# iaomw/Tracer

Measured on AMD Instinct MI355X. Metric: Mrays/s at 1920x1080x64spp, higher is better.
Workload: dtype f32

## Files before the change

### include/tracer_test_hooks.h

```cpp
#ifndef TRACER_TEST_HOOKS_H
#define TRACER_TEST_HOOKS_H

#include "tracer_abi.h"

#ifdef __cplusplus
extern "C" {
#endif

trc_status trc_debug_profile(trc_ctx* ctx, uint64_t* out, uint32_t n_sites);
trc_status trc_sppm_hash_cells(trc_ctx* ctx, const float* cells , size_t n, float hash_scale, float* out );

trc_status trc_div_by_test(trc_ctx* ctx, const float* a, const float* b, size_t n, float* fast , float* plain );
trc_status trc_unary_test(trc_ctx* ctx, uint32_t op, uint32_t first_bits, uint64_t count, uint64_t* n_mismatch, uint32_t* first_mismatch);

trc_status trc_debug_denoise_state(trc_ctx* ctx, float* integrated, float* history, float* moments);

trc_status trc_texture_sample_test(trc_ctx* ctx, uint32_t index, const float* uv , size_t n, float* rgb );

trc_status trc_debug_env_tables(trc_ctx* ctx, float* weight, uint32_t* rows, uint32_t* marg, double* total, float* build_ms);
trc_status trc_env_light_test(trc_ctx* ctx, const uint32_t* draws , size_t n, float* dir_pdf ,
                              const float* dirs , size_t m, float* pdf );

trc_status trc_debug_mesh_light_tables(trc_ctx* ctx, uint32_t* alias , uint32_t* tri , float* pdfA ,
                                       double* total, uint32_t* n_lights);
trc_status trc_mesh_light_test(trc_ctx* ctx, const uint32_t* draws , const float* pos , size_t n, uint32_t* tri ,
                               float* out );

typedef struct trc_kernel_choice {
    uint32_t shape, variant, lds_resident, triangle_materials, strip, launches;
} trc_kernel_choice;
trc_status trc_debug_last_kernel(trc_ctx* ctx, trc_kernel_choice* out);

#ifdef __cplusplus
}
#endif
#endif
```

### tracer_amd/abi.py

```python
import ctypes as C

TRC_ABI_VERSION = 13
TRC_TILE = 16
TRC_MAX_BVH_DEPTH = 64
TREE_SAH, TREE_TRIANGLE_LEAVES = 1, 2
TRC_UNIQUE_ID_BYTES = 128
DT_U8, DT_U32, DT_F32 = 1, 3, 7
OP_SUM, OP_MAX, OP_MIN = 0, 2, 3

PRIM_SPHERE, PRIM_SQUARE, PRIM_CUBE, PRIM_TRIANGLE, PRIM_BVH, PRIM_UNKNOW = range(6)
(MAT_DIFFUSE, MAT_LAMBERT, MAT_ORENNAYAR, MAT_PLASTIC, MAT_METAL, MAT_GLASS,
 MAT_ISOTROPIC, MAT_DIELECTRIC, MAT_DEMOFOX, MAT_PBR, MAT_NIL) = range(11)
TEX_CONSTANT, TEX_CHECKER, TEX_NOISE, TEX_IMAGE = range(4)
INTEGRATOR_PATH, INTEGRATOR_MIS, INTEGRATOR_VOLUME = 0, 1, 2
MEDIUM_NIL, MEDIUM_HOMOGENEOUS, MEDIUM_GRIDDENSITY = 0, 1, 2
SCENE_CORNELL, SCENE_CORNELL_SPHERES, SCENE_CORNELL_MESH, SCENE_CORNELL_VOLUME = 0, 1, 2, 3
FLAG_COLLECT_STATS = 1
FLAG_FIXED_ORDER = 2
FLAG_SOBOL = 4
FLAG_SMALL_BLOCKS, FLAG_LARGE_BLOCKS = 8, 16
FLAG_ENV_LIGHT = 32
FLAG_MESH_LIGHTS = 64
TRACE_ANY_HIT, TRACE_PRODUCTION = 1, 2
SOBOL_DIMS, SOBOL_MATRIX_SIZE = 40, 52

SHARD_SEED_STRIDE = 0x9E3779B97F4A7C15


def shard_seed(seed, sample_group):
    return (int(seed) + int(sample_group) * SHARD_SEED_STRIDE) & 0xFFFFFFFFFFFFFFFF


OK = 0
ERR_INVALID_ARG, ERR_NO_DEVICE, ERR_HIP, ERR_NO_SCENE, ERR_NO_FRAME = -1, -2, -3, -4, -5
ERR_BVH_INVALID, ERR_UNSUPPORTED, ERR_RCCL, ERR_OOM = -6, -7, -8, -9


class float2(C.Structure):
    _fields_ = [("x", C.c_float), ("y", C.c_float)]


class float3(C.Structure):
    _fields_ = [("x", C.c_float), ("y", C.c_float), ("z", C.c_float), ("_pad", C.c_float)]


class float4(C.Structure):
    _fields_ = [("x", C.c_float), ("y", C.c_float), ("z", C.c_float), ("w", C.c_float)]


class float4x4(C.Structure):
    _fields_ = [("columns", float4 * 4)]


class AABB(C.Structure):
    _fields_ = [("mini", float3), ("maxi", float3)]


class BVH(C.Structure):
    _fields_ = [("parent", C.c_uint32), ("left", C.c_uint32), ("right", C.c_uint32), ("axis", C.c_uint32),
                ("pType", C.c_int32), ("pIndex", C.c_uint32), ("_pad", C.c_uint32 * 2), ("bBOX", AABB)]


class Sphere(C.Structure):
    _fields_ = [("radius", C.c_float), ("_pad0", C.c_uint32 * 3), ("center", float3),
                ("model_matrix", float4x4), ("normal_matrix", float4x4), ("inverse_matrix", float4x4),
                ("material", C.c_uint32), ("_pad1", C.c_uint32 * 3), ("boundingBOX", AABB)]


class Square(C.Structure):
    _fields_ = [("axis_i", C.c_uint8), ("axis_j", C.c_uint8), ("_pad0", C.c_uint8 * 6),
                ("range_i", float2), ("range_j", float2),
                ("axis_k", C.c_uint8), ("_pad1", C.c_uint8 * 3), ("value_k", C.c_float),
                ("model_matrix", float4x4), ("normal_matrix", float4x4), ("inverse_matrix", float4x4),
                ("material", C.c_uint32), ("_pad2", C.c_uint32 * 3), ("boundingBOX", AABB)]


class Cube(C.Structure):
    _fields_ = [("model_matrix", float4x4), ("normal_matrix", float4x4), ("inverse_matrix", float4x4),
                ("box", AABB), ("material", C.c_uint32), ("_pad", C.c_uint32 * 3)]


class TriangleVertex(C.Structure):
    _fields_ = [("v", C.c_float * 3), ("n", C.c_float * 3), ("uv", C.c_float * 2)]


class Pose(C.Structure):
    _fields_ = [("first", C.c_uint32), ("count", C.c_uint32), ("_pad", C.c_uint32 * 2),
                ("model_matrix", float4x4), ("normal_matrix", float4x4)]


class TextureInfo(C.Structure):
    _fields_ = [("type", C.c_int32), ("textureIndex", C.c_uint32), ("_pad", C.c_uint32 * 2), ("albedo", float3)]


class Image(C.Structure):
    _fields_ = [("width", C.c_uint32), ("height", C.c_uint32), ("rgb", C.POINTER(C.c_float))]


class Material(C.Structure):
    _fields_ = [("type", C.c_int32), ("medium", C.c_int32), ("specular", C.c_uint8), ("_pad0", C.c_uint8 * 3),
                ("eta", C.c_float), ("roughness", C.c_float), ("_pad1", C.c_uint32 * 3),
                ("textureInfo", TextureInfo)]


class Camera(C.Structure):
    _fields_ = [("lookFrom", float3), ("lookAt", float3), ("viewUp", float3),
                ("vfov", C.c_float), ("aspect", C.c_float), ("aperture", C.c_float), ("lenRadius", C.c_float),
                ("focus_dist", C.c_float), ("_pad", C.c_uint32 * 3),
                ("u", float3), ("v", float3), ("w", float3),
                ("vertical", float3), ("horizontal", float3), ("cornerLowLeft", float3)]


class PhotonRecord(C.Structure):
    _fields_ = [("flux", float3), ("normal", float3), ("position", float3), ("direction", float3),
                ("step", C.c_uint8), ("active", C.c_uint8), ("_pad", C.c_uint8 * 14)]


class CameraRecord(C.Structure):
    _fields_ = [("ratio", float3), ("position", float3), ("direction", float3),
                ("valid", C.c_uint8), ("_pad0", C.c_uint8 * 15), ("alternative", float3), ("flux", float3),
                ("radius", C.c_float), ("photonCount", C.c_uint32), ("_pad1", C.c_uint32 * 2)]


class Complex(C.Structure):
    _fields_ = [("tex_size", float2), ("view_size", float2), ("running_time", C.c_float),
                ("frame_count", C.c_uint32), ("_pad0", C.c_uint32 * 2), ("photonBox", AABB),
                ("photonBoxSize", float3), ("photonInitialRadius", C.c_float), ("photonHashScale", C.c_float),
                ("totalPhotonSum", C.c_float), ("framePhotonSum", C.c_uint32)]


PHOTON_HASHN = 512


class Scene(C.Structure):
    _fields_ = [("bvhList", C.POINTER(BVH)), ("n_bvh", C.c_uint32),
                ("sphereList", C.POINTER(Sphere)), ("n_sphere", C.c_uint32),
                ("squareList", C.POINTER(Square)), ("n_square", C.c_uint32),
                ("cubeList", C.POINTER(Cube)), ("n_cube", C.c_uint32),
                ("triList", C.POINTER(TriangleVertex)), ("n_vertex", C.c_uint32),
                ("idxList", C.POINTER(C.c_uint32)), ("n_index", C.c_uint32),
                ("materials", C.POINTER(Material)), ("n_material", C.c_uint32)]


class GridDensityInfo(C.Structure):
    _fields_ = [("sigma_a", C.c_float), ("sigma_s", C.c_float), ("sigma_t", C.c_float), ("g", C.c_float),
                ("invMaxDensity", C.c_float), ("nx", C.c_uint32), ("ny", C.c_uint32), ("nz", C.c_uint32)]


PBRT_MATTE, PBRT_PLASTIC, PBRT_METAL, PBRT_MIRROR, PBRT_GLASS, PBRT_OTHER = range(6)
PBRT_SHAPE_SPHERE, PBRT_SHAPE_TRIANGLEMESH, PBRT_SHAPE_DISK, PBRT_SHAPE_CYLINDER, PBRT_SHAPE_PLYMESH = 0, 3, 6, 7, 8
PBRT_SHAPE_CONE, PBRT_SHAPE_PARABOLOID, PBRT_SHAPE_HYPERBOLOID = 9, 10, 11
PBRT_TEX_NONE, PBRT_TEX_CHECKERBOARD, PBRT_TEX_OTHER = 0, 1, 2
PBRT_TRIANGLE_MATERIALS = 1


class PbrtInfo(C.Structure):
    _fields_ = [("camera_to_world", C.c_float * 16), ("fov", C.c_float), ("lensradius", C.c_float),
                ("focaldistance", C.c_float), ("perspective", C.c_uint32), ("xres", C.c_uint32), ("yres", C.c_uint32),
                ("n_shapes", C.c_uint32), ("n_unsupported_shapes", C.c_uint32), ("n_unsupported_materials", C.c_uint32),
                ("n_triangle_material_conflicts", C.c_uint32), ("mis_ready", C.c_uint32), ("n_unsupported_textures", C.c_uint32),
                ("n_instances", C.c_uint32)]


class PbrtShape(C.Structure):
    _fields_ = [("kind", C.c_int32), ("shape_to_world", C.c_float * 16), ("radius", C.c_float),
                ("n_vertices", C.c_uint32), ("n_indices", C.c_uint32), ("material", C.c_int32), ("color", C.c_float * 3),
                ("emitter", C.c_int32), ("L", C.c_float * 3), ("mapped_type", C.c_int32), ("mapped_index", C.c_uint32),
                ("mapped_material", C.c_uint32), ("zmin", C.c_float), ("zmax", C.c_float), ("innerradius", C.c_float),
                ("phimax", C.c_float), ("texture", C.c_int32), ("tex2", C.c_float * 3), ("p1", C.c_float * 3), ("p2", C.c_float * 3)]


class Params(C.Structure):
    _fields_ = [("spp", C.c_uint32), ("max_depth", C.c_uint32), ("integrator", C.c_uint32),
                ("frame0", C.c_uint32), ("tile_rank", C.c_uint32), ("tile_nranks", C.c_uint32),
                ("flags", C.c_uint32), ("view_height", C.c_uint32)]


class Ray(C.Structure):
    _fields_ = [("origin", C.c_float * 3), ("tmax", C.c_float), ("direction", C.c_float * 3), ("_pad", C.c_uint32)]


class Hit(C.Structure):
    _fields_ = [("hit", C.c_int32), ("pType", C.c_int32), ("pIndex", C.c_uint32), ("t", C.c_float),
                ("p", C.c_float * 3), ("gn", C.c_float * 3), ("sn", C.c_float * 3), ("uv", C.c_float * 2),
                ("material", C.c_uint32), ("PDF", C.c_float),
                ("n_descend", C.c_uint32), ("n_return", C.c_uint32), ("n_leaf", C.c_uint32)]


class GBufferTexel(C.Structure):
    _fields_ = [("depth", C.c_float), ("normal", C.c_float * 3), ("albedo", C.c_float * 3), ("id", C.c_uint32)]


class DenoiseParams(C.Structure):
    _fields_ = [("flags", C.c_uint32), ("iterations", C.c_uint32), ("alpha_color", C.c_float), ("alpha_moments", C.c_float),
                ("sigma_z", C.c_float), ("normal_exponent", C.c_uint32), ("sigma_l", C.c_float), ("min_history", C.c_uint32)]


GBUFFER_MISS = 0xFFFFFFFF
DENOISE_DEMODULATE = 1
DENOISE_ALBEDO_EPS = 0.001
DENOISE_MAX_ITERATIONS = 5


class KernelChoice(C.Structure):
    _fields_ = [("shape", C.c_uint32), ("variant", C.c_uint32), ("lds_resident", C.c_uint32), ("triangle_materials", C.c_uint32),
                ("strip", C.c_uint32), ("launches", C.c_uint32)]


KERNEL_SHAPES = ("one", "strip", "pwg", "dense")
KERNEL_VARIANTS = ("plain", "stats", "sobol", "tex", "env", "env_tex", "mesh", "mesh_tex")


class LaunchShape(C.Structure):
    _fields_ = [("entries", C.c_uint32), ("wave_slots", C.c_uint32), ("longest_entry_ms", C.c_double),
                ("sum_entries_ms", C.c_double), ("work_over_slots_ms", C.c_double), ("clock_mhz", C.c_double)]


class Stats(C.Structure):
    _fields_ = [("paths", C.c_uint64), ("rays", C.c_uint64), ("shaded", C.c_uint64),
                ("n_descend", C.c_uint64), ("n_return", C.c_uint64),
                ("n_leaf_sphere", C.c_uint64), ("n_leaf_square", C.c_uint64),
                ("n_leaf_cube", C.c_uint64), ("n_leaf_triangle", C.c_uint64),
                ("n_hit_triangle", C.c_uint64), ("n_hit_cube", C.c_uint64),
                ("launches", C.c_uint64), ("kernel_ms", C.c_double), ("schedule_ms", C.c_double)]

    def as_dict(self):
        return {n: getattr(self, n) for n, _ in self._fields_}


_EXPECTED_SIZES = {float2: 8, float3: 16, float4x4: 64, AABB: 32, BVH: 64, Sphere: 272, Square: 272, Cube: 240,
                   TriangleVertex: 32, Pose: 144, TextureInfo: 32, Material: 64, Camera: 176, Ray: 32, Params: 32, GBufferTexel: 32, DenoiseParams: 32,
                   PhotonRecord: 80, CameraRecord: 112, Complex: 96}
for _t, _n in _EXPECTED_SIZES.items():
    assert C.sizeof(_t) == _n, f"{_t.__name__}: ctypes size {C.sizeof(_t)} != ABI size {_n}"

DEVICE_SYMBOLS = [
    "trc_abi_version", "trc_build_flavor", "trc_has_test_hooks", "trc_status_string", "trc_last_error", "trc_create", "trc_destroy",
    "trc_upload_scene", "trc_upload_density", "trc_upload_scene_lbvh", "trc_upload_scene_sah", "trc_upload_scene_device", "trc_download_bvh", "trc_lbvh_info", "trc_set_camera", "trc_set_environment", "trc_set_environment_map", "trc_resize", "trc_seed",
    "trc_upload_rng", "trc_download_rng", "trc_upload_accum", "trc_download_accum", "trc_clear_accum", "trc_tonemap",
    "trc_render", "trc_synchronize", "trc_trace_rays", "trc_get_stats", "trc_reset_stats",
    "trc_sppm_init", "trc_sppm_frames", "trc_sppm_download",
    "trc_device_info", "trc_device_pci_bus_id", "trc_shard_seed", "trc_group_compose_samples", "trc_group_compose_samples_async", "trc_group_unique_id", "trc_group_init", "trc_group_reduce_accum", "trc_group_reduce_accum_async", "trc_group_allreduce_mean_accum", "trc_download_composed", "trc_group_finalize",
    "trc_group_set_collectives", "trc_debug_set", "trc_debug_block_costs", "trc_debug_launch_shape", "trc_debug_primary_replays",
    "trc_denoise_default_params", "trc_denoise", "trc_download_denoised", "trc_tonemap_denoised", "trc_download_gbuffer", "trc_denoise_reset",
    "trc_upload_textures", "trc_upload_triangle_materials", "trc_update_vertices", "trc_debug_refit_ms",
    "trc_pose_vertices", "trc_download_vertices", "trc_debug_pose_overflows",
]
HOOK_SYMBOLS = ["trc_debug_profile", "trc_sppm_hash_cells", "trc_div_by_test", "trc_unary_test", "trc_debug_denoise_state", "trc_texture_sample_test",
                "trc_debug_env_tables", "trc_env_light_test", "trc_debug_mesh_light_tables", "trc_mesh_light_test", "trc_debug_last_kernel"]
HOST_SYMBOLS = [
    "trc_host_build_node", "trc_host_build_tree", "trc_host_tree_depth", "trc_host_make_camera",
    "trc_host_prepare_camera", "trc_host_fill_rng", "trc_host_scene_create", "trc_host_scene_create_leaves", "trc_host_scene_destroy",
    "trc_host_scene_view", "trc_host_scene_load_pbrt", "trc_host_mesh_load_obj", "trc_host_mesh_load_pbrt", "trc_host_mesh_load_ply", "trc_host_load_hdr", "trc_host_mesh_make_ball", "trc_host_mesh_replicate", "trc_host_mesh_from_arrays",
    "trc_host_mesh_view", "trc_host_mesh_destroy", "trc_host_make_density_info", "trc_host_make_cloud",
    "trc_host_load_density_pbrt", "trc_host_free", "trc_host_write_png", "trc_host_sobol_matrices32",
    "trc_host_sobol_interval_tables", "trc_host_load_png", "trc_host_scene_load_pbrt_flags", "trc_host_scene_triangle_materials",
]
```

### tracer_amd/csrc/trc_ctx.hpp

```cpp
#pragma once

#include <hip/hip_runtime.h>

#include <initializer_list>
#include <string>
#include <utility>
#include <vector>

#include "tracer_abi.h"
#ifdef TRC_TEST_HOOKS
#include "tracer_test_hooks.h"
#endif
#include "dev_integrator.hpp"

using namespace trcdev;

extern __shared__ __attribute__((aligned(16))) uint32_t trc_smem[];

constexpr uint32_t kLaunchCodeShift = 25u;
constexpr uint32_t kLaunchIndexMask = (1u << kLaunchCodeShift) - 1u;
constexpr uint32_t kCostSlots = 84u;
constexpr uint32_t kPlanWords = 12u;

struct KScene {
    DScene sc;
    float root_box[6];
};

struct KRender {
    KScene ks;
    DCamera cam;
    float ambient[3];
    const float* env_rgb; uint32_t env_w, env_h;
    DFrame fr;
    uint32_t spp, max_depth, frame0;
    uint32_t view_height;
    const uint32_t* tiles;
    const float* density;
    trc_GridDensityInfo dinfo;
    const uint8_t* occupancy;
    unsigned long long* stats;
    uint32_t* stack_ovf;
    uint32_t* queue;
    uint32_t blk_shift;
    uint32_t n_tiles, strip;
    const uint32_t* order;
    const uint32_t* n_launch;
    uint32_t cost_div;
    uint32_t* block_cost;
    uint32_t cost_stride;
    const uint32_t* sobol32;
    const uint64_t* sobol_vdc;
    uint32_t sobol_m;
    const float* tex_texels;
    const uint4* tex_desc;
    uint32_t n_tex;
    uint32_t* memo;
    uint32_t replay;
    uint32_t replay_chain;
};

struct KRenderEnv {
    KRender kp;
    EnvLight el;
};

struct KRenderMesh {
    KRender kp;
    MeshLight ml;
};

struct KTrace {
    KScene ks;
    const trc_ray* rays;
    trc_hit* hits;
    uint32_t n;
};

__device__ __forceinline__ const uint32_t* stage_scene(const DScene& sc) {
    const uint4* src = reinterpret_cast<const uint4*>(sc.blob);
    uint4* dst = reinterpret_cast<uint4*>(trc_smem);
    const uint32_t n16 = sc.lds_dwords >> 2;
    for (uint32_t i = threadIdx.x; i < n16; i += kBlock) dst[i] = src[i];
    __syncthreads();
    return trc_smem;
}

__device__ __forceinline__ uint32_t* lane_stack(const DScene& sc) { return trc_smem + sc.lds_dwords + threadIdx.x; }
__device__ __forceinline__ uint32_t* lane_lvstack(const DScene& sc) { return trc_smem + sc.lds_dwords + sc.stack_lds * kBlock + threadIdx.x; }

__device__ __forceinline__ SceneRef make_scene_ref(const DScene& sc, const uint32_t* small_base) {
    SceneRef S;
    S.small_base = small_base;
    S.blob = sc.blob;
    S.off_nodes = sc.off_nodes; S.off_spheres = sc.off_spheres; S.off_squares = sc.off_squares;
    S.off_cubes = sc.off_cubes; S.off_materials = sc.off_materials;
    S.off_tripos = sc.off_tripos; S.off_triattr = sc.off_triattr;
    S.n_lds_nodes = sc.n_lds_nodes;
    S.stack_lds = sc.stack_lds;
    S.stack_cap = sc.stack_depth;
    S.ovf = nullptr;
    S.descend_min = sc.descend_min;
    return S;
}

constexpr uint32_t kStatRows = 1024;
constexpr uint32_t kStatRowStride = ((kStatCount + 3 * kProfCount + 15) / 16) * 16;
static_assert(kStatRowStride <= 64, "k_stats_sum sums a row with one 64-thread workgroup");
__device__ __forceinline__ unsigned long long* stat_row(unsigned long long* stats, uint32_t wave_index) {
    return stats + (size_t)(wave_index & (kStatRows - 1u)) * kStatRowStride;
}

__device__ __forceinline__ uint32_t wave_sum(uint32_t v) {
#pragma unroll
    for (int off = 32; off > 0; off >>= 1) v += __shfl_xor(v, off, 64);
    return v;
}


struct SppmState;
struct DenoiseState;

struct trc_ctx {
    int device = -1;
    hipStream_t stream = nullptr;
    hipEvent_t ev_start = nullptr, ev_stop = nullptr;
    std::string error;

    bool has_scene = false;
    KScene ks{};
    uint32_t* d_blob = nullptr;
    size_t blob_bytes = 0;
    bool lds_scene = false;
    bool lds_prefix_ok = false;
    uint32_t* d_stack_ovf = nullptr;
    size_t stack_ovf_bytes = 0;
    uint32_t* d_memo = nullptr;
    size_t memo_bytes = 0;
    uint32_t* d_queue = nullptr;
    trc_BVH* d_bvh_ref = nullptr;
    uint32_t n_bvh_ref = 0, lbvh_height = 0;
    float lbvh_build_ms = 0.0f;
    trc_TriangleVertex* d_verts = nullptr; uint32_t* d_idx = nullptr; uint32_t n_vertex = 0;
    uint32_t* d_refit_parent = nullptr;
    uint32_t* d_refit_refnode = nullptr;
    uint32_t* d_refit_arrive = nullptr;
    float* d_refit_root = nullptr;
    std::vector<uint32_t> refit_levels;
    float refit_ms = 0.0f;
    hipEvent_t refit_ev[3] = {nullptr, nullptr, nullptr};
    bool refit_pending = false;
    trc_TriangleVertex* d_rest = nullptr;
    trc_pose* d_pose_table = nullptr; size_t pose_table_bytes = 0;
    uint32_t pose_count_seen = 0;
    uint32_t pose_overflows = 0;
    bool refit_posed = false;
    float* d_density = nullptr;
    uint8_t* d_occupancy = nullptr;
    trc_GridDensityInfo dinfo{};

    bool has_camera = false;
    DCamera cam{};
    float ambient[3] = {0, 0, 0};
    float* d_envmap = nullptr; uint32_t env_w = 0, env_h = 0;
    uint32_t* d_sobol32 = nullptr; uint64_t* d_sobol_vdc = nullptr; uint32_t sobol_m = ~0u;
    float* d_tex_texels = nullptr; uint4* d_tex_desc = nullptr; uint32_t n_tex = 0; uint32_t scene_min_image = ~0u;
    bool tex_active() const { return scene_min_image < n_tex; }
    bool tri_materials = false;
    uint8_t* d_envl = nullptr; double envl_total = 0.0; float envl_build_ms = 0.0f;
    Light cost_light = Light::None;
    uint8_t* d_meshl = nullptr; bool mesh_built = false; uint32_t mesh_n_lights = 0; double mesh_total = 0.0;

    uint32_t width = 0, height = 0;
    uint32_t* d_rng = nullptr;
    float* d_accum = nullptr;

    uint32_t* d_tiles = nullptr;
    uint32_t* d_block_cost = nullptr;
    uint32_t* d_order_keys[2] = {nullptr, nullptr};
    uint32_t* d_order_vals[2] = {nullptr, nullptr};
    uint32_t* d_order_hist = nullptr;
    uint32_t* d_split = nullptr;
    uint32_t* d_whole = nullptr;
    uint32_t* d_cost_est = nullptr;
    uint32_t* d_qsplit = nullptr;
    uint32_t* d_qwhole = nullptr;
    uint32_t* d_swhole = nullptr;
    uint32_t* d_launch = nullptr;
    uint32_t* d_plan = nullptr;
    uint32_t* d_cost_scratch = nullptr;
    uint32_t* d_plan_gather = nullptr;
    uint32_t plan_streak = 0, plan_reused = 0, plan_n = 0, plan_wave_slots = 0, plan_grid_cap = 0; bool plan_split_mode = false;
    uint32_t launch_cap = 0;
    bool split_live = false;
    bool cost_quarters = false;
    bool cost_valid = false; uint32_t cost_strip = 1;
    uint32_t last_cost_div = 0, last_wave_slots = 0;
    struct LastKernel { uint32_t shape = 0, variant = 0, lds_resident = 0, tri_materials = 0, strip = 0, count = 0; } last_kernel;
    trc_params deferred{}; bool has_deferred = false; uint64_t deferred_calls = 0;
    int cost_head_age = 0;
    bool cost_fresh_next = false;
    uint32_t cost_integrator = 0xFFFFFFFFu;
    const uint32_t* d_stale_order = nullptr;
    const uint32_t* d_last_order = nullptr; uint32_t order_age = 0;
    int cu_count = 0;
    uint32_t n_tiles = 0, tiles_nranks = 0, tiles_rank = 0, tiles_view_height = 0, tiles_blk_shift = 3;

    unsigned long long* d_stats = nullptr;
    unsigned long long* d_stats_sum = nullptr;
    uint64_t launches = 0;
    double kernel_ms = 0.0;
    double schedule_ms = 0.0;
    std::vector<std::pair<hipEvent_t, hipEvent_t>> pending_sched;
    std::vector<std::pair<hipEvent_t, hipEvent_t>> pending;
    std::vector<hipEvent_t> event_pool;

    void* comm = nullptr;
    int nranks = 1, rank = 0;
    float* d_reduce_recv = nullptr;
    float* d_accum_alt = nullptr;
    float* d_composed = nullptr;
    hipStream_t comm_stream = nullptr;
    hipEvent_t ev_rendered = nullptr, ev_busy = nullptr, ev_busy_alt = nullptr;
    bool busy = false, busy_alt = false;
    float* d_shard_in = nullptr; float* d_shard_out = nullptr; size_t shard_px = 0; int shard_nranks = 0;
    float* d_shard_src = nullptr; hipEvent_t ev_snapshot_free = nullptr; bool snapshot_busy = false;

    SppmState* sppm = nullptr;
    DenoiseState* denoise = nullptr;

    trc_collectives coll{};
    bool coll_active = false;
    void* h_stage = nullptr;
    size_t h_stage_bytes = 0;
    uint32_t* h_readback = nullptr;
    char* h_xfer = nullptr;
    hipEvent_t ev_xfer[2] = {nullptr, nullptr};

    struct Knobs {
        int no_lds_fit = 0;
        int stack_lds_levels = 0;
        int strip_len = 0;
        int no_pwg = 0;
        int sppm_serial_camera = 0;
        int sppm_timing = 0;
        int force_blk_shift = 0;
        int no_split = 0;
        int no_cost_filter = 0;
        int no_cold_probe = 0;
        int probe_spp = 0;
        int no_plan_reuse = 0;
        int no_coalesce = 0;
        int no_dense = 0;
        int head_stages = 0;
        int descend_min = 0;
        int camera_policy = 0;
        int no_primary_replay = 0;
        int replay_min_lanes = 0;
        int replay_chain = 0;
        int mesh_light_pick = 1;
        int refit_single = 0;
        int strip_force = 0;
    } knobs;
    std::vector<const void*> lds_granted;

    bool grouped() const { return comm != nullptr || coll_active; }
};


inline trc_status trc_fail(trc_ctx* ctx, trc_status s, const std::string& msg) {
    if (ctx) ctx->error = msg;
    return s;
}
#define HIP_TRY(ctx, expr)                                                                 \
    do {                                                                                   \
        hipError_t e_ = (expr);                                                            \
        if (e_ != hipSuccess)                                                              \
            return trc_fail(ctx, e_ == hipErrorOutOfMemory ? TRC_ERR_OOM : TRC_ERR_HIP,     \
                            std::string(#expr) + ": " + hipGetErrorString(e_));            \
    } while (0)

#define TRC_TRY(expr)                                                                      \
    do {                                                                                   \
        const trc_status s_ = (expr);                                                      \
        if (s_ != TRC_OK) return s_;                                                       \
    } while (0)

struct DevBuf {
    void* p = nullptr;
    DevBuf() = default;
    DevBuf(DevBuf&& o) noexcept : p(o.release()) {}
    DevBuf(const DevBuf&) = delete;
    DevBuf& operator=(const DevBuf&) = delete;
    ~DevBuf() { (void)hipFree(p); }
    trc_status alloc(trc_ctx* ctx, size_t bytes, const char* what) {
        if (hipMalloc(&p, bytes) == hipSuccess) return TRC_OK;
        p = nullptr;
        (void)hipGetLastError();
        return trc_fail(ctx, TRC_ERR_OOM, std::string("hipMalloc ") + what);
    }
    template <class T> T* as() const { return static_cast<T*>(p); }
    void* release() { void* q = p; p = nullptr; return q; }
};

struct DevBufs {
    std::vector<DevBuf> bufs;
    template <class T> trc_status alloc(trc_ctx* ctx, T** out, size_t count, const char* what) {
        bufs.emplace_back();
        TRC_TRY(bufs.back().alloc(ctx, (count ? count : 1) * sizeof(T), what));
        *out = bufs.back().as<T>();
        return TRC_OK;
    }
};

template <class T>
inline trc_status trc_grow_buffer(trc_ctx* ctx, T*& buf, size_t& have, size_t need, const char* msg) {
    if (need <= have) return TRC_OK;
    HIP_TRY(ctx, hipStreamSynchronize(ctx->stream));
    (void)hipFree(buf); buf = nullptr;
    have = 0;
    if (hipMalloc((void**)&buf, need) != hipSuccess) return trc_fail(ctx, TRC_ERR_OOM, msg);
    have = need;
    return TRC_OK;
}

struct IdBlob { char internal[TRC_UNIQUE_ID_BYTES]; };
struct Rccl {
    void* handle = nullptr;
    bool ready = false;
    int (*GetUniqueId)(void*) = nullptr;
    int (*CommInitRank)(void**, int, IdBlob, int) = nullptr;
    int (*Reduce)(const void*, void*, size_t, int, int, int, void*, hipStream_t) = nullptr;
    int (*AllReduce)(const void*, void*, size_t, int, int, void*, hipStream_t) = nullptr;
    int (*AllGather)(const void*, void*, size_t, int, void*, hipStream_t) = nullptr;
    int (*Send)(const void*, size_t, int, int, void*, hipStream_t) = nullptr;
    int (*Recv)(void*, size_t, int, int, void*, hipStream_t) = nullptr;
    int (*GroupStart)() = nullptr;
    int (*GroupEnd)() = nullptr;
    int (*CommDestroy)(void*) = nullptr;
    const char* (*GetErrorString)(int) = nullptr;
};
extern Rccl g_rccl;
bool trc_load_rccl(std::string& err);
constexpr int kNcclUint8 = 1, kNcclUint32 = 3, kNcclFloat = 7, kNcclSum = 0, kNcclMax = 2, kNcclMin = 3;

trc_status trc_coll_reduce(trc_ctx* ctx, void* buf, size_t count, int dtype, int op, int root, hipStream_t st, const char* what);
trc_status trc_coll_allreduce(trc_ctx* ctx, void* buf, size_t count, int dtype, int op, hipStream_t st, const char* what);
trc_status trc_coll_allgather(trc_ctx* ctx, void* buf, size_t bytes_per_rank, hipStream_t st, const char* what);

constexpr size_t kXferChunk = 4u << 20;
trc_status trc_copy_to_host(trc_ctx* ctx, void* host, const void* dev, size_t bytes, hipStream_t st);
trc_status trc_copy_to_device(trc_ctx* ctx, void* dev, const void* host, size_t bytes, hipStream_t st);
struct trc_read_item { void* host; const void* dev; size_t bytes; };
trc_status trc_read_to_host(trc_ctx* ctx, hipStream_t st, const char* what, std::initializer_list<trc_read_item> items);

trc_status trc_ensure_tiles(trc_ctx* ctx, uint32_t nranks, uint32_t rank, uint32_t view_height = 0, uint32_t blk_shift = 3);
size_t trc_dyn_lds_bytes(const trc_ctx* ctx, bool stats);
void trc_sort_pairs24(hipStream_t st, uint32_t* keys[2], uint32_t* vals[2], uint32_t* hist, uint32_t* digit_base, uint32_t n, int* result);
uint32_t trc_sort_hist_words(uint32_t n);
trc_status trc_tonemap_plane(trc_ctx* ctx, const float* plane, uint8_t* rgba8, float* exposure_out);
trc_status trc_flush(trc_ctx* ctx);
hipEvent_t trc_get_event(trc_ctx* ctx);
struct TimedSection {
    trc_ctx* ctx; hipStream_t st; hipEvent_t e0, e1;
    TimedSection(trc_ctx* c, hipStream_t s) : ctx(c), st(s), e0(trc_get_event(c)), e1(trc_get_event(c)) { if (e0 && e1) (void)hipEventRecord(e0, st); }
    ~TimedSection() { if (e0) ctx->event_pool.push_back(e0); if (e1) ctx->event_pool.push_back(e1); }
    void stop() { if (e0 && e1) (void)hipEventRecord(e1, st); }
    float ms() const { float v = 0.0f; return e0 && e1 && hipEventElapsedTime(&v, e0, e1) == hipSuccess ? v : 0.0f; }
};
void trc_sppm_release(trc_ctx* ctx);
void trc_denoise_release(trc_ctx* ctx);
inline uint32_t trc_scene_min_image(const trc_scene* s) {
    uint32_t m = ~0u;
    for (uint32_t i = 0; i < s->n_material; ++i)
        if (s->materials[i].textureInfo.type == TRC_TEX_IMAGE && s->materials[i].textureInfo.textureIndex < m) m = s->materials[i].textureInfo.textureIndex;
    return m;
}
void trc_denoise_invalidate(trc_ctx* ctx);
trc_status trc_env_light_build(trc_ctx* ctx);
void trc_env_light_free(trc_ctx* ctx);
EnvLight trc_env_light_view(const trc_ctx* ctx);
trc_status trc_mesh_light_build(trc_ctx* ctx);
void trc_mesh_light_free(trc_ctx* ctx);
MeshLight trc_mesh_light_view(const trc_ctx* ctx);
constexpr size_t kReadbackBytes = 1024;
inline trc_status trc_readback_alloc(trc_ctx* ctx) {
    if (!ctx->h_readback) HIP_TRY(ctx, hipHostMalloc((void**)&ctx->h_readback, kReadbackBytes, hipHostMallocDefault));
    return TRC_OK;
}
trc_status trc_refit_settle_pending(trc_ctx* ctx);
inline trc_status trc_refit_settle(trc_ctx* ctx) { return ctx->refit_pending ? trc_refit_settle_pending(ctx) : TRC_OK; }
void trc_refit_free(trc_ctx* ctx);
void trc_sppm_order_after_camera(trc_ctx* ctx);

inline void trc_forget_costs(trc_ctx* ctx) { ctx->cost_valid = false; ctx->d_last_order = nullptr; ctx->d_stale_order = nullptr; }
inline void trc_picture_changed(trc_ctx* ctx) { trc_denoise_invalidate(ctx); }
enum SceneChange { kSceneReplaced, kSceneMaterials, kSceneVerticesMoved };
void trc_scene_changed(trc_ctx* ctx, SceneChange kind);
void trc_release_scene(trc_ctx* ctx);
void trc_adopt_scene(trc_ctx* ctx, KScene ks, const trc_scene* s);
void trc_release_frame(trc_ctx* ctx);
void trc_release_tiles(trc_ctx* ctx);
void trc_collect_finished_events(trc_ctx* ctx);
trc_status trc_read_stats_sum(trc_ctx* ctx, unsigned long long* h, size_t count);
```

### tracer_amd/csrc/trc_hooks.hip

```cpp
#include <hip/hip_runtime.h>

#include <string>

#include "trc_ctx.hpp"

extern "C" int trc_has_test_hooks(void) {
#ifdef TRC_TEST_HOOKS
    return 1;
#else
    return 0;
#endif
}

#ifdef TRC_TEST_HOOKS
__global__ void __launch_bounds__(256) k_div_by_test(const float* a, const float* b, uint32_t n, float* fast, float* plain) {
    const uint32_t i = blockIdx.x * 256u + threadIdx.x;
    if (i >= n) return;
    const float av = a[i], bv = b[i];
    const GuardedDivBy d = guarded_div_by(bv);
    const F3 q = guarded_div(f3(av, -av, av * 0.75f), d);
    fast[3 * i] = q.x; fast[3 * i + 1] = q.y; fast[3 * i + 2] = q.z;
    plain[3 * i] = av / bv; plain[3 * i + 1] = -av / bv; plain[3 * i + 2] = (av * 0.75f) / bv;
}

__global__ void __launch_bounds__(256) k_unary_test(uint32_t op, uint32_t first, uint64_t count, unsigned long long* out) {
    unsigned long long bad = 0, first_bad = ~0ull;
    for (uint64_t i = (uint64_t)blockIdx.x * 256u + threadIdx.x; i < count; i += (uint64_t)gridDim.x * 256u) {
        const uint32_t bits = first + (uint32_t)i;
        const float x = __uint_as_float(bits);
        float a, b;
        if (op == 0u) { a = rcp_cr(x); b = 1.0f / x; }
        else if (op == 1u) { a = sqrt_cr(x); b = sqrtf(x); }
#if TRC_WAVE_GUARDS
        else if (op == 3u) { a = div_const(x, div_by_pi()); b = x / kPi; }
        else if (op == 4u) { a = div_const(x, div_by_sqr001()); b = x / (0.01f * 0.01f); }
        else if (op == 5u) { a = div_const(x, div_by_sqr002()); b = x / (0.02f * 0.02f); }
        else if (op == 6u) { a = div_const(x, div_by_sqr01()); b = x / (0.1f * 0.1f); }
#endif
        else { a = rsqrt_cr(x); b = 1.0f / sqrtf(x); }
        const bool same = __float_as_uint(a) == __float_as_uint(b) || (a != a && b != b);
        if (!same) { bad++; first_bad = min(first_bad, (unsigned long long)bits); }
    }
    if (bad) { atomicAdd(&out[0], bad); atomicMin(&out[1], first_bad); }
}

extern "C" {
trc_status trc_debug_profile(trc_ctx* ctx, uint64_t* out, uint32_t n_sites) {
    TRC_TRY(trc_flush(ctx));
    if (!ctx || !out) return TRC_ERR_INVALID_ARG;
    HIP_TRY(ctx, hipSetDevice(ctx->device));
    unsigned long long h[kStatCount + 3 * kProfCount];
    TRC_TRY(trc_read_stats_sum(ctx, h, kStatCount + 3 * kProfCount));
    for (uint32_t i = 0; i < n_sites && i < (uint32_t)kProfCount; ++i)
        for (int k = 0; k < 3; ++k) out[3 * i + k] = h[kStatCount + 3 * i + k];
    return TRC_OK;
}

__global__ void __launch_bounds__(256) k_texture_sample_test(const float* texels, const uint4* desc, uint32_t n_tex, uint32_t index,
                                                             const float* uv, uint32_t n, float* rgb) {
    const uint32_t i = blockIdx.x * 256u + threadIdx.x;
    if (i >= n) return;
    TexTable tt; tt.texels = texels; tt.desc = desc; tt.n = n_tex;
    F2 p; p.x = uv[2 * i]; p.y = uv[2 * i + 1];
    const F3 c = image_sample(tt, index, p);
    rgb[3 * i] = c.x; rgb[3 * i + 1] = c.y; rgb[3 * i + 2] = c.z;
}
trc_status trc_texture_sample_test(trc_ctx* ctx, uint32_t index, const float* uv, size_t n, float* rgb) {
    TRC_TRY(trc_flush(ctx));
    if (!ctx || (n && (!uv || !rgb))) return TRC_ERR_INVALID_ARG;
    if (index >= ctx->n_tex) return trc_fail(ctx, TRC_ERR_INVALID_ARG, "trc_texture_sample_test: no such image");
    if (n == 0) return TRC_OK;
    if (n > 0x7FFFFFFFu / 3u) return trc_fail(ctx, TRC_ERR_INVALID_ARG, "trc_texture_sample_test: too many pairs in one call");
    HIP_TRY(ctx, hipSetDevice(ctx->device));
    DevBuf d;
    TRC_TRY(d.alloc(ctx, n * 5 * sizeof(float), "texture sample test"));
    float *d_uv = d.as<float>(), *d_rgb = d_uv + 2 * n;
    TRC_TRY(trc_copy_to_device(ctx, d_uv, uv, n * 8, ctx->stream));
    hipLaunchKernelGGL(k_texture_sample_test, dim3((unsigned)((n + 255) / 256)), dim3(256), 0, ctx->stream,
                       ctx->d_tex_texels, ctx->d_tex_desc, ctx->n_tex, index, d_uv, (uint32_t)n, d_rgb);
    const hipError_t e = hipGetLastError();
    if (e != hipSuccess) return trc_fail(ctx, TRC_ERR_HIP, std::string("trc_texture_sample_test: ") + hipGetErrorString(e));
    return trc_copy_to_host(ctx, rgb, d_rgb, n * 12, ctx->stream);
}

trc_status trc_debug_last_kernel(trc_ctx* ctx, trc_kernel_choice* out) {
    TRC_TRY(trc_flush(ctx));
    if (!ctx || !out) return TRC_ERR_INVALID_ARG;
    const trc_ctx::LastKernel& k = ctx->last_kernel;
    out->shape = k.shape; out->variant = k.variant; out->lds_resident = k.lds_resident; out->triangle_materials = k.tri_materials;
    out->strip = k.strip; out->launches = k.count;
    return TRC_OK;
}

trc_status trc_div_by_test(trc_ctx* ctx, const float* a, const float* b, size_t n, float* fast, float* plain) {
    if (!ctx || (n && (!a || !b || !fast || !plain))) return TRC_ERR_INVALID_ARG;
    if (n == 0) return TRC_OK;
    if (n > 0x7FFFFFFFu / 3u) return trc_fail(ctx, TRC_ERR_INVALID_ARG, "trc_div_by_test: too many pairs in one call");
    HIP_TRY(ctx, hipSetDevice(ctx->device));
    DevBuf d;
    TRC_TRY(d.alloc(ctx, n * 8 * sizeof(float), "div_by test"));
    float *d_a = d.as<float>(), *d_b = d_a + n, *d_fast = d_a + 2 * n, *d_plain = d_a + 5 * n;
    TRC_TRY(trc_copy_to_device(ctx, d_a, a, n * 4, ctx->stream));
    TRC_TRY(trc_copy_to_device(ctx, d_b, b, n * 4, ctx->stream));
    hipLaunchKernelGGL(k_div_by_test, dim3((unsigned)((n + 255) / 256)), dim3(256), 0, ctx->stream, d_a, d_b, (uint32_t)n, d_fast, d_plain);
    const hipError_t e = hipGetLastError();
    if (e != hipSuccess) return trc_fail(ctx, TRC_ERR_HIP, std::string("trc_div_by_test: ") + hipGetErrorString(e));
    TRC_TRY(trc_copy_to_host(ctx, fast, d_fast, n * 12, ctx->stream));
    return trc_copy_to_host(ctx, plain, d_plain, n * 12, ctx->stream);
}

trc_status trc_unary_test(trc_ctx* ctx, uint32_t op, uint32_t first_bits, uint64_t count, uint64_t* n_mismatch, uint32_t* first_mismatch) {
    if (!ctx || !n_mismatch || op > 6u || count > (1ull << 32)) return TRC_ERR_INVALID_ARG;
    HIP_TRY(ctx, hipSetDevice(ctx->device));
    DevBuf buf;
    TRC_TRY(buf.alloc(ctx, 16, "unary test"));
    unsigned long long* const d = buf.as<unsigned long long>();
    unsigned long long h[2] = {0ull, ~0ull};
    TRC_TRY(trc_copy_to_device(ctx, d, h, 16, ctx->stream));
    if (count) hipLaunchKernelGGL(k_unary_test, dim3(ctx->cu_count * 16), dim3(256), 0, ctx->stream, op, first_bits, count, d);
    TRC_TRY(trc_read_to_host(ctx, ctx->stream, "trc_unary_test", {{h, d, 16}}));
    *n_mismatch = h[0];
    if (first_mismatch) *first_mismatch = (uint32_t)h[1];
    return TRC_OK;
}

}
#endif
```

### tracer_amd/csrc/trc_render_config.hpp

```cpp
#pragma once

#include "trc_ctx.hpp"

#ifndef TRC_MIS_HYBRID
#define TRC_MIS_HYBRID 1
#endif
#ifndef TRC_VOLUME_HYBRID
#define TRC_VOLUME_HYBRID 0
#endif
constexpr bool hybrid_stack(int integrator) {
    return integrator == TRC_INTEGRATOR_PATH || (integrator == TRC_INTEGRATOR_MIS ? TRC_MIS_HYBRID != 0 : TRC_VOLUME_HYBRID != 0);
}
#ifndef TRC_DEFER_LDS
#define TRC_DEFER_LDS 0
#endif
#ifndef TRC_DEFER_GLOBAL
#define TRC_DEFER_GLOBAL 1
#endif

#ifndef TRC_PATH_WAVES
#define TRC_PATH_WAVES 5
#endif
#ifndef TRC_PATH_WAVES_DENSE
#define TRC_PATH_WAVES_DENSE 6
#endif
#ifndef TRC_DENSE_MIN_BLOCKS_PER_SLOT
#define TRC_DENSE_MIN_BLOCKS_PER_SLOT 4
#endif
#ifndef TRC_PATH_WAVES_GLOBAL
#define TRC_PATH_WAVES_GLOBAL 7
#endif
#ifndef TRC_MIS_WAVES
#define TRC_MIS_WAVES 8
#endif
#ifndef TRC_MIS_WAVES_LDS
#define TRC_MIS_WAVES_LDS 8
#endif
#ifndef TRC_VOLUME_WAVES
#define TRC_VOLUME_WAVES 4
#endif
#ifndef TRC_PWG_WAVES_PATH
#define TRC_PWG_WAVES_PATH 4
#endif
#ifndef TRC_PWG_PER_CU_PATH
#define TRC_PWG_PER_CU_PATH 7
#endif
#ifndef TRC_PWG_WAVES_MIS
#define TRC_PWG_WAVES_MIS 16
#endif
#ifndef TRC_PWG_PER_CU_MIS
#define TRC_PWG_PER_CU_MIS 2
#endif
#ifndef TRC_PWG_WAVES_VOLUME
#define TRC_PWG_WAVES_VOLUME 16
#endif
#ifndef TRC_PWG_PER_CU_VOLUME
#define TRC_PWG_PER_CU_VOLUME 1
#endif
#ifndef TRC_STRIP_PATH_WAVES
#define TRC_STRIP_PATH_WAVES 4
#endif
constexpr int pwg_waves(int integrator) { return integrator == TRC_INTEGRATOR_PATH ? TRC_PWG_WAVES_PATH : (integrator == TRC_INTEGRATOR_MIS ? TRC_PWG_WAVES_MIS : TRC_PWG_WAVES_VOLUME); }
enum : uint32_t { kParkCachedX = 0, kParkCachedY, kParkCachedZ, kParkU, kParkV, kParkSample, kParkRays, kParkShaded, kParkPx, kParkPy };
#ifndef TRC_PARK_PATH
#define TRC_PARK_PATH 8
#endif
#ifndef TRC_PARK_MIS
#define TRC_PARK_MIS 0
#endif
#ifndef TRC_PARK_VOLUME
#define TRC_PARK_VOLUME 10
#endif
#ifndef TRC_PARK_DENSE
#define TRC_PARK_DENSE 0
#endif
constexpr uint32_t pwg_park_rows(int integrator) { return integrator == TRC_INTEGRATOR_PATH ? TRC_PARK_PATH : (integrator == TRC_INTEGRATOR_MIS ? TRC_PARK_MIS : TRC_PARK_VOLUME); }
static_assert((TRC_PARK_PATH == 0 || TRC_PARK_PATH == 8 || TRC_PARK_PATH == 10) && (TRC_PARK_MIS == 0 || TRC_PARK_MIS == 8 || TRC_PARK_MIS == 10) &&
              (TRC_PARK_VOLUME == 0 || TRC_PARK_VOLUME == 8 || TRC_PARK_VOLUME == 10) && (TRC_PARK_DENSE == 0 || TRC_PARK_DENSE == 8 || TRC_PARK_DENSE == 10), "park rows: 0, 8 or 10");
enum : uint32_t { kMemoPx = 0, kMemoPy, kMemoPz, kMemoNx, kMemoNy, kMemoNz, kMemoTag, kMemoMat, kMemoU, kMemoV };
constexpr uint32_t kMemoNone = 0xFFFFFFFFu;
constexpr uint32_t kMemoSameSide = 0x80000000u;
#ifndef TRC_REPLAY_DENSE
#define TRC_REPLAY_DENSE 8
#endif
#ifndef TRC_REPLAY_DENSE_GLOBAL
#define TRC_REPLAY_DENSE_GLOBAL 0
#endif
#ifndef TRC_REPLAY_PWG_PATH
#define TRC_REPLAY_PWG_PATH 10
#endif
#ifndef TRC_REPLAY_MIN_LANES
#define TRC_REPLAY_MIN_LANES 1
#endif
#ifndef TRC_REPLAY_CHAIN
#define TRC_REPLAY_CHAIN 1
#endif
static_assert((TRC_REPLAY_DENSE == 0 || TRC_REPLAY_DENSE == 8 || TRC_REPLAY_DENSE == 10) && (TRC_REPLAY_PWG_PATH == 0 || TRC_REPLAY_PWG_PATH == 10), "memo rows: 0, 8 or 10 (10 wherever image textures may be live)");
constexpr uint32_t dense_lds_rows() { return (uint32_t)TRC_PARK_DENSE + (TRC_REPLAY_DENSE_GLOBAL ? 0u : (uint32_t)TRC_REPLAY_DENSE); }
constexpr uint32_t pwg_memo_rows(int integrator) { return integrator == TRC_INTEGRATOR_PATH ? (uint32_t)TRC_REPLAY_PWG_PATH : 0u; }
#ifndef TRC_PWG_STACK_LDS_PATH
#define TRC_PWG_STACK_LDS_PATH (TRC_PARK_PATH == 10 ? 10 : (TRC_PARK_PATH == 8 ? 12 : 16))
#endif
#ifndef TRC_PWG_STACK_LDS_MIS
#define TRC_PWG_STACK_LDS_MIS 8
#endif
#ifndef TRC_PWG_STACK_LDS_VOLUME
#define TRC_PWG_STACK_LDS_VOLUME 16
#endif
constexpr uint32_t pwg_stack_lds_levels(int integrator) { return integrator == TRC_INTEGRATOR_MIS ? TRC_PWG_STACK_LDS_MIS : (integrator == TRC_INTEGRATOR_PATH ? TRC_PWG_STACK_LDS_PATH : TRC_PWG_STACK_LDS_VOLUME); }
constexpr int pwg_per_cu(int integrator) { return integrator == TRC_INTEGRATOR_PATH ? TRC_PWG_PER_CU_PATH : (integrator == TRC_INTEGRATOR_MIS ? TRC_PWG_PER_CU_MIS : TRC_PWG_PER_CU_VOLUME); }

constexpr int render_waves(bool lds, bool stats, int integrator) {
    return stats ? 1 : integrator == TRC_INTEGRATOR_VOLUME ? TRC_VOLUME_WAVES
                     : integrator == TRC_INTEGRATOR_MIS ? (lds ? TRC_MIS_WAVES_LDS : TRC_MIS_WAVES) : (lds ? TRC_PATH_WAVES : TRC_PATH_WAVES_GLOBAL);
}
constexpr int strip_waves(int integrator) { return integrator == TRC_INTEGRATOR_VOLUME ? 3 : (integrator == TRC_INTEGRATOR_PATH ? TRC_STRIP_PATH_WAVES : 4); }
constexpr int pwg_simd_waves(int integrator) { return pwg_waves(integrator) * pwg_per_cu(integrator) / 4; }

enum RenderArgs { kArgsPlain, kArgsEnv, kArgsMesh };
struct RenderKernel {
    const void* fn;
    int waves;
    RenderArgs args;
};
inline RenderKernel render_kernel(void (*fn)(KRender), int waves) { return {reinterpret_cast<const void*>(fn), waves, kArgsPlain}; }
inline RenderKernel render_kernel(void (*fn)(KRenderEnv), int waves) { return {reinterpret_cast<const void*>(fn), waves, kArgsEnv}; }
inline RenderKernel render_kernel(void (*fn)(KRenderMesh), int waves) { return {reinterpret_cast<const void*>(fn), waves, kArgsMesh}; }
enum RenderVariant { kVariantPlain, kVariantStats, kVariantSobol, kVariantTex, kVariantEnv, kVariantEnvTex, kVariantMesh, kVariantMeshTex, kVariants };
struct RenderKernels {
    RenderKernel one[kVariants];
    RenderKernel strip[kVariants];
    RenderKernel pwg[kVariants];
};
extern const RenderKernels render_lds_path, render_lds_mis, render_lds_volume, render_mem_path, render_mem_mis, render_mem_volume;
extern const RenderKernel render_dense;
namespace trimat {
extern const RenderKernels render_lds_path, render_lds_mis, render_lds_volume, render_mem_path, render_mem_mis, render_mem_volume;
extern const RenderKernel render_dense;
}
```

### tracer_amd/csrc/trc_render_kernels.hpp

```cpp
#pragma once

#include <hip/hip_runtime.h>

#include "trc_render_config.hpp"

#if TRC_TRIANGLE_MATERIALS
#define TRC_RENDER_NS_BEGIN namespace trimat {
#define TRC_RENDER_NS_END }
#else
#define TRC_RENDER_NS_BEGIN
#define TRC_RENDER_NS_END
#endif
TRC_RENDER_NS_BEGIN

template <bool TEX, class CX>
__device__ __forceinline__ void set_ctx_tex(CX& cx, const KRender& kp) {
    if constexpr (TEX) { cx.tex.texels = kp.tex_texels; cx.tex.desc = kp.tex_desc; cx.tex.n = kp.n_tex; }
}
template <Light LIGHT, class CX>
__device__ __forceinline__ void set_ctx_light(CX& cx, const LightTables<LIGHT>* tables) {
    if constexpr (LIGHT != Light::None) cx.light = *tables;
}
template <bool SOBOL, bool TEX, Light LIGHT>
__device__ __forceinline__ void fill_path_ctx(PathCtxOf<TEX, LIGHT>& cx, const KRender& kp, const DScene& sc, const uint32_t* small_base,
                                              uint32_t* stack, uint32_t* lvstack, const LightTables<LIGHT>* tables) {
    cx.S = make_scene_ref(sc, small_base);
    cx.root_min = f3(kp.ks.root_box[0], kp.ks.root_box[1], kp.ks.root_box[2]);
    cx.root_max = f3(kp.ks.root_box[3], kp.ks.root_box[4], kp.ks.root_box[5]);
    cx.sh.mats = small_base + sc.off_materials;
    set_ctx_tex<TEX>(cx, kp);
    set_ctx_light<LIGHT>(cx, tables);
    cx.ambient = f3(kp.ambient[0], kp.ambient[1], kp.ambient[2]);
    cx.env.rgb = kp.env_rgb; cx.env.w = kp.env_w; cx.env.h = kp.env_h;
    cx.stack = stack;
    cx.lvstack = lvstack;
    cx.max_depth = kp.max_depth;
    cx.density = kp.density;
    cx.dinfo = kp.dinfo;
    cx.occupancy = kp.occupancy;
    if (SOBOL) {
        cx.sobol32 = kp.sobol32; cx.sobol_vdc = kp.sobol_vdc;
        cx.sobol_m = kp.sobol_m; cx.sobol_res = 1u << kp.sobol_m;
    }
}
template <bool LDS, bool STATS, int INTEGRATOR, bool SOBOL, bool HYB, int PARK = 0, bool TEX = false, Light LIGHT = Light::None, int MEMO = 0, class COUNT = uint32_t>
__device__ __forceinline__ void render_block(const KRender& kp, const DScene& sc, const uint32_t* small_base, uint32_t* stack, uint32_t* lvstack,
                                             uint32_t* ovf, uint32_t* park, const uint32_t slot, const uint32_t lane,
                                             COUNT& n_rays, COUNT& n_shaded, uint32_t& n_paths, TravCounters& cnt,
                                             const LightTables<LIGHT>* tables = nullptr, uint32_t* memo = nullptr) {
    static_assert(MEMO == 0 || (INTEGRATOR == TRC_INTEGRATOR_PATH && !STATS && !SOBOL && LIGHT == Light::None), "primary replay: tracePath production kernels");
    static_assert(MEMO == 0 || MEMO == 10 || !TEX, "an image texture reads rec.uv: 10 memo rows");
    uint32_t replays = 0;
    const uint64_t t_start = clock64();
    const uint32_t entry = kp.order ? kp.order[slot] : slot;
    const uint32_t index = entry & kLaunchIndexMask, code = entry >> kLaunchCodeShift;
    if (index >= kp.n_tiles) return;
    const uint32_t tile = kp.tiles[index];
    const uint32_t part = code >= 21u ? (code - 21u) >> 2 : (code >= 5u ? code - 5u : 0u);
    const uint32_t quarter = code >= 5u ? part >> 2 : (code ? code - 1u : 0u);
    const uint32_t bs = code >= 21u ? 0u : (code >= 5u ? 1u : (code ? 2u : kp.blk_shift));
    const uint32_t pixel = code >= 21u ? (code - 21u) & 3u : 0u;
    const uint32_t qx = code ? ((quarter & 1u) << 2) + (code >= 5u ? (part & 1u) << 1 : 0u) + (pixel & 1u) : 0u;
    const uint32_t qy = code ? ((quarter >> 1) << 2) + (code >= 5u ? ((part >> 1) & 1u) << 1 : 0u) + (pixel >> 1) : 0u;
    const uint32_t px = ((tile & 0xFFFFu) << kp.blk_shift) + qx + (lane & ((1u << bs) - 1u));
    const uint32_t py = ((tile >> 16) << kp.blk_shift) + qy + (lane >> bs);
    const uint32_t W = kp.fr.width, H = kp.fr.height;
    const bool active = lane < (1u << (2u * bs)) && px < W && py < H;
    const uint32_t canon = index * kp.cost_stride + (code ? code - 1u : 0u);

    if (active) {
        PathCtxOf<TEX, LIGHT> cx;
        fill_path_ctx<SOBOL, TEX, LIGHT>(cx, kp, sc, small_base, stack, lvstack, tables);
        cx.S.ovf = ovf;
        if (SOBOL) { cx.sobol_xy[0] = px; cx.sobol_xy[1] = py % kp.view_height; }

        F3 cached_r = f3(0);
        float u_r = 0, v_r = 0;
        uint32_t s_r = 0;
        size_t pix_r = 0;
        auto row_f = [&](uint32_t r) { return __uint_as_float(park[r * kBlock]); };
        auto put_f = [&](uint32_t r, float x) { park[r * kBlock] = __float_as_uint(x); };
        auto get_cached = [&]() { if constexpr (PARK) return f3(row_f(kParkCachedX), row_f(kParkCachedY), row_f(kParkCachedZ)); else return cached_r; };
        auto set_cached = [&](F3 c) { if constexpr (PARK) { put_f(kParkCachedX, c.x); put_f(kParkCachedY, c.y); put_f(kParkCachedZ, c.z); } else cached_r = c; };
        auto get_sample = [&]() { if constexpr (PARK) return park[kParkSample * kBlock]; else return s_r; };
        auto set_sample = [&](uint32_t s) { if constexpr (PARK) park[kParkSample * kBlock] = s; else s_r = s; };
        uint4 texel;
        {
            const size_t pix = (size_t)py * W + px;
            texel = reinterpret_cast<const uint4*>(kp.fr.rng)[pix];
            const float4 acc = reinterpret_cast<const float4*>(kp.fr.accum)[pix];
            const float u = (float)px / (float)W;
            const float v = (float)(py % kp.view_height) / (float)kp.view_height;
            set_cached(f3(acc.x, acc.y, acc.z));
            set_sample(0u);
            if constexpr (PARK) { put_f(kParkU, u); put_f(kParkV, v); }
            if constexpr (PARK >= 10) { park[kParkPx * kBlock] = px; park[kParkPy * kBlock] = py; }
            else { u_r = u; v_r = v; pix_r = pix; }
        }

        PathState ps;
        Pcg rng;
        uint64_t state_after_cast = 0;
        const bool replay_on = MEMO != 0 && kp.replay != 0u;
        bool first = replay_on, have = false, terminal = false;
        auto memo_f = [&](uint32_t r) { return __uint_as_float(memo[r * kBlock]); };
        auto at_eye = [&](const F3& o) {
            return __float_as_uint(o.x) == __float_as_uint(kp.cam.lookFrom[0]) && __float_as_uint(o.y) == __float_as_uint(kp.cam.lookFrom[1]) &&
                   __float_as_uint(o.z) == __float_as_uint(kp.cam.lookFrom[2]);
        };
        auto begin_sample = [&](uint32_t s) {
            const float u = PARK ? row_f(kParkU) : u_r, v = PARK ? row_f(kParkV) : v_r;
            path_begin(ps, cast_ray(kp.cam, u, v, rng), kp.max_depth);
            if constexpr (MEMO != 0) {
                if (replay_on && s != 0u) {
                    const uint32_t mat = memo[kMemoMat * kBlock];
                    if (mat != kMemoNone) {
                        if (at_eye(ps.ray.o)) {
                            const uint32_t tag = memo[kMemoTag * kBlock];
                            if (tag == kTagNone) terminal = true;
                            else {
                                ps.rec.p = f3(memo_f(kMemoPx), memo_f(kMemoPy), memo_f(kMemoPz));
                                ps.rec.gn = f3(memo_f(kMemoNx), memo_f(kMemoNy), memo_f(kMemoNz));
                                ps.rec.sn = (mat & kMemoSameSide) ? ps.rec.gn : -ps.rec.gn;
                                ps.rec.material = mat & ~kMemoSameSide;
                                ps.rec.tag = tag;
                                if constexpr (MEMO >= 10) { ps.rec.uv.x = memo_f(kMemoU); ps.rec.uv.y = memo_f(kMemoV); }
                                have = true;
                            }
                            bump(n_rays);
                        } else {
                            memo[kMemoMat * kBlock] = kMemoNone; memo[kMemoTag * kBlock] = s - 1u;
                        }
                    }
                }
            }
            if (SOBOL) {
                state_after_cast = rng.state;
                ps.sobol_index = sobol_interval_to_index(cx, (uint64_t)(kp.frame0 + s));
                ps.sobol_dim = 0;
            }
        };
        bool alive = kp.spp > 0;
        if (alive) {
            rng.state = ((uint64_t)texel.z << 32) | texel.w;
            rng.inc = ((uint64_t)texel.x << 32) | texel.y;
            begin_sample(0u);
        }
        auto finish_sample = [&](F3 color) {
            ProfScope<STATS> scope(cnt, kProfFinish);
            for (;;) {
                const bool bad = is_inf(color.x) || is_nan(color.x) || is_inf(color.y) || is_nan(color.y) ||
                                 is_inf(color.z) || is_nan(color.z);
                if (bad) color = f3(0);
                uint32_t s = get_sample();
                const uint32_t frame = kp.frame0 + s;
                set_cached(div_shared(get_cached() * (float)frame + color, (float)(frame + 1)));
                if (SOBOL) rng.state = state_after_cast;
                if constexpr (!PARK) {
                    texel.y = (uint32_t)rng.state; texel.x = (uint32_t)(rng.state >> 32);
                    texel.w = (uint32_t)rng.inc;   texel.z = (uint32_t)(rng.inc >> 32);
                    n_paths++;
                }
                ++s;
                set_sample(s);
                if (s == kp.spp) {
                    alive = false;
                } else {
                    if constexpr (PARK) { const uint64_t t = rng.state; rng.state = rng.inc; rng.inc = t; }
                    else {
                        rng.state = ((uint64_t)texel.z << 32) | texel.w;
                        rng.inc = ((uint64_t)texel.x << 32) | texel.y;
                    }
                    begin_sample(s);
                }
                if constexpr (MEMO != 0) {
                    if (terminal) { terminal = false; color = f3(memo_f(kMemoPx), memo_f(kMemoPy), memo_f(kMemoPz)); continue; }
                }
                break;
            }
        };
        auto memo_store = [&](bool hitted) {
            uint32_t mat = kMemoNone, tag = 0u;
            bool ends = false;
            if (at_eye(ps.ray.o)) {
                ends = !hitted || mat_type(cx.sh, ps.rec.material) == kMatDiffuse;
                if (ends) { mat = 0u; tag = kTagNone; }
                else {
                    const bool uv_read = MEMO < 10 && (ps.rec.tag >> kTagIndexBits) >= 2u && mat_tex(cx.sh, ps.rec.material) == kTexChecker;
                    if (!uv_read && ps.rec.material < kMemoSameSide - 1u) {
                        const bool same = __float_as_uint(ps.rec.sn.x) == __float_as_uint(ps.rec.gn.x);
                        mat = ps.rec.material | (same ? kMemoSameSide : 0u); tag = ps.rec.tag;
                        memo[kMemoPx * kBlock] = __float_as_uint(ps.rec.p.x); memo[kMemoPy * kBlock] = __float_as_uint(ps.rec.p.y);
                        memo[kMemoPz * kBlock] = __float_as_uint(ps.rec.p.z);
                        memo[kMemoNx * kBlock] = __float_as_uint(ps.rec.gn.x); memo[kMemoNy * kBlock] = __float_as_uint(ps.rec.gn.y);
                        memo[kMemoNz * kBlock] = __float_as_uint(ps.rec.gn.z);
                        if constexpr (MEMO >= 10) { memo[kMemoU * kBlock] = __float_as_uint(ps.rec.uv.x); memo[kMemoV * kBlock] = __float_as_uint(ps.rec.uv.y); }
                    }
                }
            }
            memo[kMemoMat * kBlock] = mat; memo[kMemoTag * kBlock] = tag;
            return ends;
        };
        uint32_t drained = 0;
        while (alive) {
            ProfScope<STATS> loop_scope(cnt, kProfLoop);
            constexpr bool kVolume = INTEGRATOR == TRC_INTEGRATOR_VOLUME;
            constexpr int kDefer = STATS ? 0 : (LDS ? TRC_DEFER_LDS : TRC_DEFER_GLOBAL);
            bool hitted = true;
            bool drain = false, ends = false;
            if constexpr (MEMO != 0) {
                drain = (uint32_t)__popcll(__ballot(have)) >= kp.replay && drained < kp.replay_chain && replay_on;
                drained = drain ? drained + 1u : 0u;
            }
            if (!drain && !have && !(kVolume && TRC_TRACK_SLICE > 0 && ps.tracking)) {
                bump(n_rays);
                hitted = scene_hit<LDS, STATS, false, false, kVolume, HYB, kDefer>(cx.S, cx.root_min, cx.root_max, ps.ray, ps.rec, FLT_MAX,
                                                                                  cx.stack, cx.lvstack, cnt);
                if constexpr (MEMO != 0) {
                    if (first) { ends = memo_store(hitted); first = false; }
                }
            }
            if (!drain || have) {
                have = false;
                F3 color;
                const bool finished = (INTEGRATOR == TRC_INTEGRATOR_PATH)
                                          ? path_step<STATS, SOBOL, TEX>(cx, ps, hitted, rng, cnt, n_shaded, color)
                                          : mis_step<LDS, STATS, kVolume, SOBOL, HYB, TEX, LIGHT>(cx, ps, hitted, rng, cnt, n_rays, n_shaded, color);
                if constexpr (MEMO != 0) {
                    if (ends) { memo[kMemoPx * kBlock] = __float_as_uint(color.x); memo[kMemoPy * kBlock] = __float_as_uint(color.y); memo[kMemoPz * kBlock] = __float_as_uint(color.z); }
                }
                if (finished) finish_sample(color);
            }
        }
        if constexpr (MEMO != 0) {
            if (replay_on) replays = memo[kMemoMat * kBlock] != kMemoNone ? kp.spp - 1u : memo[kMemoTag * kBlock];
        }
        if constexpr (PARK) {
            n_paths += kp.spp;
            texel.y = (uint32_t)rng.state; texel.x = (uint32_t)(rng.state >> 32);
            texel.w = (uint32_t)rng.inc;   texel.z = (uint32_t)(rng.inc >> 32);
        }
        const F3 cached = get_cached();
        size_t pix = pix_r;
        if constexpr (PARK >= 10) pix = (size_t)park[kParkPy * kBlock] * W + park[kParkPx * kBlock];
        else if constexpr (PARK != 0) {
            const uint32_t entry2 = kp.order ? *reinterpret_cast<const volatile uint32_t*>(kp.order + slot) : slot;
            const uint32_t code2 = entry2 >> kLaunchCodeShift;
            const uint32_t tile2 = *reinterpret_cast<const volatile uint32_t*>(kp.tiles + (entry2 & kLaunchIndexMask));
            const uint32_t part2 = code2 >= 21u ? (code2 - 21u) >> 2 : (code2 >= 5u ? code2 - 5u : 0u);
            const uint32_t quarter2 = code2 >= 5u ? part2 >> 2 : (code2 ? code2 - 1u : 0u);
            const uint32_t bs2 = code2 >= 21u ? 0u : (code2 >= 5u ? 1u : (code2 ? 2u : kp.blk_shift));
            const uint32_t pixel2 = code2 >= 21u ? (code2 - 21u) & 3u : 0u;
            const uint32_t qx2 = code2 ? ((quarter2 & 1u) << 2) + (code2 >= 5u ? (part2 & 1u) << 1 : 0u) + (pixel2 & 1u) : 0u;
            const uint32_t qy2 = code2 ? ((quarter2 >> 1) << 2) + (code2 >= 5u ? ((part2 >> 1) & 1u) << 1 : 0u) + (pixel2 >> 1) : 0u;
            pix = (size_t)(((tile2 >> 16) << kp.blk_shift) + qy2 + (lane >> bs2)) * W + ((tile2 & 0xFFFFu) << kp.blk_shift) + qx2 + (lane & ((1u << bs2) - 1u));
        }
        float4 out; out.x = cached.x; out.y = cached.y; out.z = cached.z; out.w = 1.0f;
        reinterpret_cast<float4*>(kp.fr.accum)[pix] = out;
        reinterpret_cast<uint4*>(kp.fr.rng)[pix] = texel;
    }

    if (lane == 0) kp.block_cost[canon] = (uint32_t)min((unsigned long long)(clock64() - t_start) / kp.cost_div, 0xFFFFFFull);
    if constexpr (MEMO != 0) {
        const uint32_t r_replays = wave_sum(replays);
        if (lane == 0 && r_replays) atomicAdd(&stat_row(kp.stats, slot)[kStatReplays], (unsigned long long)r_replays);
    }
}

template <bool LDS, bool STATS, int INTEGRATOR, bool SOBOL, int PARK = 0, bool TEX = false, Light LIGHT = Light::None, int MEMO = 0, bool MEMO_GLOBAL = false>
__device__ __forceinline__ void render_workgroup(const KRender& kp, const LightTables<LIGHT>* tables = nullptr) {
    if (kp.n_launch && blockIdx.x >= *kp.n_launch) return;
    const DScene& sc = kp.ks.sc;
    const uint32_t* small_base = stage_scene(sc);
    uint32_t* stack = lane_stack(sc);
    uint32_t* lvstack = lane_lvstack(sc);

    const uint32_t lane = threadIdx.x;
    uint32_t n_rays = 0, n_shaded = 0, n_paths = 0;
    TravCounters cnt;
    counters_zero(cnt);
    constexpr bool kHybridStack = !LDS && !STATS && hybrid_stack(INTEGRATOR);
    uint32_t* ovf = kHybridStack ? kp.stack_ovf + (size_t)blockIdx.x * sc.stack_ovf_rows * kBlock + lane : nullptr;
    uint32_t* memo = nullptr;
    if constexpr (MEMO != 0 && MEMO_GLOBAL) memo = kp.memo + (size_t)blockIdx.x * MEMO * kBlock + lane;
    else if constexpr (MEMO != 0) memo = stack + (sc.stack_lds + PARK) * kBlock;
    if constexpr (PARK != 0) {
        uint32_t* park = stack + sc.stack_lds * kBlock;
        park[kParkRays * kBlock] = 0u; park[kParkShaded * kBlock] = 0u;
        LdsCount c_rays{park + kParkRays * kBlock}, c_shaded{park + kParkShaded * kBlock};
        render_block<LDS, STATS, INTEGRATOR, SOBOL, kHybridStack, PARK, TEX, LIGHT, MEMO>(kp, sc, small_base, stack, lvstack, ovf, park, blockIdx.x, lane, c_rays, c_shaded, n_paths, cnt, tables, memo);
        n_rays = park[kParkRays * kBlock]; n_shaded = park[kParkShaded * kBlock];
    } else
    render_block<LDS, STATS, INTEGRATOR, SOBOL, kHybridStack, 0, TEX, LIGHT, MEMO>(kp, sc, small_base, stack, lvstack, ovf, nullptr, blockIdx.x, lane, n_rays, n_shaded, n_paths, cnt, tables, memo);

    uint32_t r_paths = wave_sum(n_paths), r_rays = wave_sum(n_rays), r_shaded = wave_sum(n_shaded);
    unsigned long long* const stats = stat_row(kp.stats, blockIdx.x);
    if (lane == 0) {
        atomicAdd(&stats[kStatPaths], (unsigned long long)r_paths);
        atomicAdd(&stats[kStatRays], (unsigned long long)r_rays);
        atomicAdd(&stats[kStatShaded], (unsigned long long)r_shaded);
    }
    if (STATS) {
        uint32_t v[8] = {cnt.n_descend, cnt.n_return, cnt.leaf[0], cnt.leaf[1], cnt.leaf[2], cnt.leaf[3],
                         cnt.hit_triangle, cnt.hit_cube};
        const int slot[8] = {kStatDescend, kStatReturn, kStatLeafSphere, kStatLeafSquare, kStatLeafCube,
                             kStatLeafTriangle, kStatHitTriangle, kStatHitCube};
#pragma unroll
        for (int i = 0; i < 8; ++i) {
            uint32_t r = wave_sum(v[i]);
            if (lane == 0) atomicAdd(&stats[slot[i]], (unsigned long long)r);
        }
        for (int i = 0; i < kProfCount; ++i) {
            uint32_t rl = wave_sum(cnt.prof_lane[i]), rw = wave_sum(cnt.prof_wave[i]);
            unsigned long long rc = cnt.prof_cycles[i];
#pragma unroll
            for (int off = 32; off > 0; off >>= 1) rc += __shfl_xor(rc, off);
            if (lane == 0) {
                atomicAdd(&stats[kStatCount + 3 * i], (unsigned long long)rl);
                atomicAdd(&stats[kStatCount + 3 * i + 1], (unsigned long long)rw);
                atomicAdd(&stats[kStatCount + 3 * i + 2], rc);
            }
        }
    }
}
template <bool LDS, bool STATS, int INTEGRATOR, bool SOBOL>
__global__ void __launch_bounds__(kBlock, render_waves(LDS, STATS, INTEGRATOR)) k_render(const KRender kp) { render_workgroup<LDS, STATS, INTEGRATOR, SOBOL>(kp); }
template <bool LDS, int INTEGRATOR>
__global__ void __launch_bounds__(kBlock, render_waves(LDS, false, INTEGRATOR)) k_render_tex(const KRender kp) { render_workgroup<LDS, false, INTEGRATOR, false, 0, true>(kp); }
template <bool LDS, int INTEGRATOR, bool TEX>
__global__ void __launch_bounds__(kBlock, render_waves(LDS, false, INTEGRATOR)) k_render_env(const KRenderEnv kpe) {
    render_workgroup<LDS, false, INTEGRATOR, false, 0, TEX, Light::Env>(kpe.kp, &kpe.el);
}
template <bool LDS, int INTEGRATOR, bool TEX>
__global__ void __launch_bounds__(kBlock, render_waves(LDS, false, INTEGRATOR)) k_render_mesh(const KRenderMesh kpm) {
    render_workgroup<LDS, false, INTEGRATOR, false, 0, TEX, Light::Mesh>(kpm.kp, &kpm.ml);
}

template <int INTEGRATOR, bool SOBOL>
__global__ void __launch_bounds__(64 * pwg_waves(INTEGRATOR), pwg_simd_waves(INTEGRATOR)) k_render_pwg(const KRender kp) {
    constexpr bool TEX = false;
    constexpr Light LIGHT = Light::None;
    const void* const tables = nullptr;
#include "trc_render_pwg_body.inc"
}
template <int INTEGRATOR>
__global__ void __launch_bounds__(64 * pwg_waves(INTEGRATOR), pwg_simd_waves(INTEGRATOR)) k_render_pwg_tex(const KRender kp) {
    constexpr bool SOBOL = false, TEX = true;
    constexpr Light LIGHT = Light::None;
    const void* const tables = nullptr;
#include "trc_render_pwg_body.inc"
}
template <int INTEGRATOR, bool TEX>
__global__ void __launch_bounds__(64 * pwg_waves(INTEGRATOR), pwg_simd_waves(INTEGRATOR)) k_render_pwg_env(const KRenderEnv kpe) {
    constexpr bool SOBOL = false;
    constexpr Light LIGHT = Light::Env;
    const KRender& kp = kpe.kp;
    const EnvLight* const tables = &kpe.el;
#include "trc_render_pwg_body.inc"
}

template <int INTEGRATOR, bool TEX>
__global__ void __launch_bounds__(64 * pwg_waves(INTEGRATOR), pwg_simd_waves(INTEGRATOR)) k_render_pwg_mesh(const KRenderMesh kpm) {
    constexpr bool SOBOL = false;
    constexpr Light LIGHT = Light::Mesh;
    const KRender& kp = kpm.kp;
    const MeshLight* const tables = &kpm.ml;
#include "trc_render_pwg_body.inc"
}

template <bool LDS, int INTEGRATOR, bool SOBOL>
__global__ void __launch_bounds__(kBlock, strip_waves(INTEGRATOR)) k_render_strip(const KRender kp) {
    constexpr bool TEX = false;
    constexpr Light LIGHT = Light::None;
    const void* const tables = nullptr;
#include "trc_render_strip_body.inc"
}
template <bool LDS, int INTEGRATOR>
__global__ void __launch_bounds__(kBlock, strip_waves(INTEGRATOR)) k_render_strip_tex(const KRender kp) {
    constexpr bool SOBOL = false, TEX = true;
    constexpr Light LIGHT = Light::None;
    const void* const tables = nullptr;
#include "trc_render_strip_body.inc"
}
template <bool LDS, int INTEGRATOR, bool TEX>
__global__ void __launch_bounds__(kBlock, strip_waves(INTEGRATOR)) k_render_strip_env(const KRenderEnv kpe) {
    constexpr bool SOBOL = false;
    constexpr Light LIGHT = Light::Env;
    const KRender& kp = kpe.kp;
    const EnvLight* const tables = &kpe.el;
#include "trc_render_strip_body.inc"
}

template <bool LDS, int INTEGRATOR, bool TEX>
__global__ void __launch_bounds__(kBlock, strip_waves(INTEGRATOR)) k_render_strip_mesh(const KRenderMesh kpm) {
    constexpr bool SOBOL = false;
    constexpr Light LIGHT = Light::Mesh;
    const KRender& kp = kpm.kp;
    const MeshLight* const tables = &kpm.ml;
#include "trc_render_strip_body.inc"
}

template <bool LDS, int INTEGRATOR>
inline RenderKernels render_kernels() {
    constexpr bool kSobol = INTEGRATOR != TRC_INTEGRATOR_VOLUME;
    RenderKernels t{};
    t.one[kVariantPlain] = render_kernel(&k_render<LDS, false, INTEGRATOR, false>, render_waves(LDS, false, INTEGRATOR));
    t.one[kVariantStats] = render_kernel(&k_render<LDS, true, INTEGRATOR, false>, render_waves(LDS, true, INTEGRATOR));
    t.one[kVariantTex] = render_kernel(&k_render_tex<LDS, INTEGRATOR>, render_waves(LDS, false, INTEGRATOR));
    t.strip[kVariantPlain] = render_kernel(&k_render_strip<LDS, INTEGRATOR, false>, strip_waves(INTEGRATOR));
    t.strip[kVariantTex] = render_kernel(&k_render_strip_tex<LDS, INTEGRATOR>, strip_waves(INTEGRATOR));
    if constexpr (kSobol) {
        t.one[kVariantSobol] = render_kernel(&k_render<LDS, false, INTEGRATOR, true>, render_waves(LDS, false, INTEGRATOR));
        t.strip[kVariantSobol] = render_kernel(&k_render_strip<LDS, INTEGRATOR, true>, strip_waves(INTEGRATOR));
    }
    if constexpr (!LDS) {
        t.pwg[kVariantPlain] = render_kernel(&k_render_pwg<INTEGRATOR, false>, pwg_simd_waves(INTEGRATOR));
        t.pwg[kVariantTex] = render_kernel(&k_render_pwg_tex<INTEGRATOR>, pwg_simd_waves(INTEGRATOR));
        if constexpr (kSobol) t.pwg[kVariantSobol] = render_kernel(&k_render_pwg<INTEGRATOR, true>, pwg_simd_waves(INTEGRATOR));
    }
    if constexpr (INTEGRATOR == TRC_INTEGRATOR_MIS) {
        t.one[kVariantEnv] = render_kernel(&k_render_env<LDS, INTEGRATOR, false>, render_waves(LDS, false, INTEGRATOR));
        t.one[kVariantEnvTex] = render_kernel(&k_render_env<LDS, INTEGRATOR, true>, render_waves(LDS, false, INTEGRATOR));
        t.strip[kVariantEnv] = render_kernel(&k_render_strip_env<LDS, INTEGRATOR, false>, strip_waves(INTEGRATOR));
        t.strip[kVariantEnvTex] = render_kernel(&k_render_strip_env<LDS, INTEGRATOR, true>, strip_waves(INTEGRATOR));
        if constexpr (!LDS) {
            t.pwg[kVariantEnv] = render_kernel(&k_render_pwg_env<INTEGRATOR, false>, pwg_simd_waves(INTEGRATOR));
            t.pwg[kVariantEnvTex] = render_kernel(&k_render_pwg_env<INTEGRATOR, true>, pwg_simd_waves(INTEGRATOR));
        }
        t.one[kVariantMesh] = render_kernel(&k_render_mesh<LDS, INTEGRATOR, false>, render_waves(LDS, false, INTEGRATOR));
        t.one[kVariantMeshTex] = render_kernel(&k_render_mesh<LDS, INTEGRATOR, true>, render_waves(LDS, false, INTEGRATOR));
        t.strip[kVariantMesh] = render_kernel(&k_render_strip_mesh<LDS, INTEGRATOR, false>, strip_waves(INTEGRATOR));
        t.strip[kVariantMeshTex] = render_kernel(&k_render_strip_mesh<LDS, INTEGRATOR, true>, strip_waves(INTEGRATOR));
        if constexpr (!LDS) {
            t.pwg[kVariantMesh] = render_kernel(&k_render_pwg_mesh<INTEGRATOR, false>, pwg_simd_waves(INTEGRATOR));
            t.pwg[kVariantMeshTex] = render_kernel(&k_render_pwg_mesh<INTEGRATOR, true>, pwg_simd_waves(INTEGRATOR));
        }
    }
    return t;
}
TRC_RENDER_NS_END
```

### tracer_amd/csrc/trc_render_pass.hip

```cpp
#include <hip/hip_runtime.h>

#include <algorithm>
#include <cstring>
#include <string>
#include <vector>

#include "trc_launch.hpp"

static size_t dyn_lds_bytes(const DScene& sc, bool stats) {
    size_t dwords = sc.lds_dwords + (size_t)sc.stack_lds * kBlock * (stats ? 2u : 1u);
    return dwords * 4;
}
size_t trc_dyn_lds_bytes(const trc_ctx* ctx, bool stats) { return dyn_lds_bytes(ctx->ks.sc, stats); }

constexpr uint32_t kStackLdsLevels = 16;
static void set_hybrid_stack(DScene& sc, uint32_t levels) {
    sc.stack_lds = std::min(sc.stack_depth, std::max(1u, levels));
    sc.stack_ovf_rows = sc.stack_depth - sc.stack_lds;
}
static void plan_launch_lds(const trc_ctx* ctx, DScene& sc, uint32_t waves_per_simd, bool hybrid) {
    const uint32_t levels = ctx->knobs.stack_lds_levels > 0 ? (uint32_t)ctx->knobs.stack_lds_levels : kStackLdsLevels;
    if (hybrid) set_hybrid_stack(sc, ctx->knobs.no_lds_fit ? std::max(levels, sc.stack_depth) : levels);
    if (ctx->knobs.no_lds_fit) return;
    if (!ctx->lds_prefix_ok) return;
    const uint32_t per_wg = ((160u * 1024u / 4u) / (4u * waves_per_simd)) & ~127u;
    const uint32_t stack = sc.stack_lds * kBlock;
    uint32_t room = std::max(per_wg > stack ? per_wg - stack : 0u, sc.off_nodes + kNodeDwords);
    room = std::min(room, kLdsSceneBytes / 4);
    sc.n_lds_nodes = std::min(sc.n_nodes, (room - sc.off_nodes) / kNodeDwords);
    sc.lds_dwords = sc.off_nodes + sc.n_lds_nodes * kNodeDwords;
}

static bool plan_pwg_lds(const trc_ctx* ctx, DScene& sc, uint32_t waves, uint32_t per_cu, bool hybrid, uint32_t default_levels, uint32_t park_rows) {
    uint32_t levels = ctx->knobs.stack_lds_levels > 0 ? (uint32_t)ctx->knobs.stack_lds_levels : default_levels;
    const uint32_t per_wg = ((160u * 1024u / 4u) / per_cu) & ~127u;
    for (;; --levels) {
        DScene t = sc;
        if (hybrid) set_hybrid_stack(t, levels);
        const uint32_t stacks = waves * (t.stack_lds + park_rows) * kBlock;
        if (per_wg >= stacks + t.off_nodes + kNodeDwords) {
            t.n_lds_nodes = std::min(t.n_nodes, (per_wg - stacks - t.off_nodes) / kNodeDwords);
            t.lds_dwords = t.off_nodes + t.n_lds_nodes * kNodeDwords;
            sc = t;
            return true;
        }
        if (!hybrid || levels <= 6u || ctx->knobs.stack_lds_levels > 0) return false;
    }
}

namespace {

trc_status ensure_sobol_tables(trc_ctx* ctx, uint32_t m) {
    if (!ctx->d_sobol_vdc) {
        std::vector<uint32_t> m32(TRC_SOBOL_DIMS * TRC_SOBOL_MATRIX_SIZE);
        trc_sobol_matrices32(m32.data());
        if (!ctx->d_sobol32) HIP_TRY(ctx, hipMalloc((void**)&ctx->d_sobol32, m32.size() * sizeof(uint32_t)));
        TRC_TRY(trc_copy_to_device(ctx, ctx->d_sobol32, m32.data(), m32.size() * sizeof(uint32_t), ctx->stream));
        HIP_TRY(ctx, hipMalloc((void**)&ctx->d_sobol_vdc, 2 * TRC_SOBOL_MATRIX_SIZE * sizeof(uint64_t)));
        ctx->sobol_m = ~0u;
    }
    if (ctx->sobol_m != m) {
        uint64_t tb[2 * TRC_SOBOL_MATRIX_SIZE] = {};
        if (m != 0 && trc_sobol_interval_tables(m, tb, tb + TRC_SOBOL_MATRIX_SIZE) != 0)
            return trc_fail(ctx, TRC_ERR_UNSUPPORTED, "Sobol interval tables");
        HIP_TRY(ctx, hipStreamSynchronize(ctx->stream));
        TRC_TRY(trc_copy_to_device(ctx, ctx->d_sobol_vdc, tb, sizeof(tb), ctx->stream));
        ctx->sobol_m = m;
    }
    return TRC_OK;
}

const RenderKernels& render_family(bool lds_scene, uint32_t integrator, bool tri_materials) {
    static const RenderKernels* const lds[3] = {&render_lds_path, &render_lds_mis, &render_lds_volume};
    static const RenderKernels* const mem[3] = {&render_mem_path, &render_mem_mis, &render_mem_volume};
    static const RenderKernels* const lds_tm[3] = {&trimat::render_lds_path, &trimat::render_lds_mis, &trimat::render_lds_volume};
    static const RenderKernels* const mem_tm[3] = {&trimat::render_mem_path, &trimat::render_mem_mis, &trimat::render_mem_volume};
    return *(tri_materials ? (lds_scene ? lds_tm : mem_tm) : (lds_scene ? lds : mem))[integrator];
}

hipError_t launch_render(trc_ctx* ctx, const RenderLaunch& r) {
    const void* const fn = r.kern.fn;
    if (r.lds > 64 * 1024 && std::find(ctx->lds_granted.begin(), ctx->lds_granted.end(), fn) == ctx->lds_granted.end()) {
        const hipError_t e = hipFuncSetAttribute(fn, hipFuncAttributeMaxDynamicSharedMemorySize, (int)(160 * 1024));
        if (e != hipSuccess) return e;
        ctx->lds_granted.push_back(fn);
    }
    KRenderEnv kpe;
    KRenderMesh kpm;
    void* params = const_cast<KRender*>(&r.kp);
    if (r.kern.args == kArgsEnv) { kpe.kp = r.kp; kpe.el = r.el; params = &kpe; }
    if (r.kern.args == kArgsMesh) { kpm.kp = r.kp; kpm.ml = r.ml; params = &kpm; }
    void* args[] = {params};
    const hipError_t e = hipLaunchKernel(fn, dim3(r.grid), dim3(r.block), args, r.lds, ctx->stream);
    const hipError_t last = hipGetLastError();
    return e != hipSuccess ? e : last;
}

}

static trc_status render_pass(trc_ctx* ctx, const trc_params* p, bool inner);

constexpr uint32_t kColdHeadSpp = 8;
static trc_status render_check(trc_ctx* ctx, const trc_params* p, uint32_t* sobol_m = nullptr) {
    if (!ctx || !p) return TRC_ERR_INVALID_ARG;
    if (!ctx->has_scene) return trc_fail(ctx, TRC_ERR_NO_SCENE, "trc_render before trc_upload_scene");
    if (!ctx->d_accum) return trc_fail(ctx, TRC_ERR_NO_FRAME, "trc_render before trc_resize");
    if (!ctx->has_camera) return trc_fail(ctx, TRC_ERR_INVALID_ARG, "trc_render before trc_set_camera");
    const uint32_t nranks = p->tile_nranks ? p->tile_nranks : 1;
    if (p->tile_rank >= nranks) return trc_fail(ctx, TRC_ERR_INVALID_ARG, "tile_rank >= tile_nranks");
    if (p->integrator > TRC_INTEGRATOR_VOLUME) return trc_fail(ctx, TRC_ERR_INVALID_ARG, "unknown integrator");
    const bool env_light = (p->flags & TRC_FLAG_ENV_LIGHT) != 0;
    if (env_light) {
        if (p->integrator != TRC_INTEGRATOR_MIS) return trc_fail(ctx, TRC_ERR_UNSUPPORTED, "TRC_FLAG_ENV_LIGHT: traceMIS only");
        if (p->flags & (TRC_FLAG_SOBOL | TRC_FLAG_COLLECT_STATS))
            return trc_fail(ctx, TRC_ERR_UNSUPPORTED, "TRC_FLAG_ENV_LIGHT: no TRC_FLAG_SOBOL / TRC_FLAG_COLLECT_STATS kernels");
        if (!ctx->d_envmap) return trc_fail(ctx, TRC_ERR_UNSUPPORTED, "TRC_FLAG_ENV_LIGHT: no environment map (trc_set_environment_map)");
    }
    const bool mesh_lights = (p->flags & TRC_FLAG_MESH_LIGHTS) != 0;
    if (mesh_lights) {
        if (p->integrator != TRC_INTEGRATOR_MIS) return trc_fail(ctx, TRC_ERR_UNSUPPORTED, "TRC_FLAG_MESH_LIGHTS: traceMIS only");
        if (p->flags & (TRC_FLAG_SOBOL | TRC_FLAG_COLLECT_STATS | TRC_FLAG_ENV_LIGHT))
            return trc_fail(ctx, TRC_ERR_UNSUPPORTED, "TRC_FLAG_MESH_LIGHTS: no TRC_FLAG_SOBOL / TRC_FLAG_COLLECT_STATS / TRC_FLAG_ENV_LIGHT kernels");
    }
    if (p->integrator != TRC_INTEGRATOR_PATH && ctx->ks.sc.n_squares < 7 && !env_light && !mesh_lights)
        return trc_fail(ctx, TRC_ERR_INVALID_ARG, "traceMIS / traceVolume sample squareList[5] and [6] (Render.metal:320-324,172-176)");
    if (ctx->tex_active() && (p->flags & (TRC_FLAG_SOBOL | TRC_FLAG_COLLECT_STATS)))
        return trc_fail(ctx, TRC_ERR_UNSUPPORTED, "image textures: no TRC_FLAG_SOBOL / TRC_FLAG_COLLECT_STATS kernels (trc_upload_textures)");
    if (p->flags & TRC_FLAG_SOBOL) {
        if (p->integrator == TRC_INTEGRATOR_VOLUME || (p->flags & TRC_FLAG_COLLECT_STATS))
            return trc_fail(ctx, TRC_ERR_UNSUPPORTED, "TRC_FLAG_SOBOL: tracePath / traceMIS, production kernels only");
        if (2ull * p->max_depth > TRC_SOBOL_DIMS)
            return trc_fail(ctx, TRC_ERR_UNSUPPORTED, "TRC_FLAG_SOBOL: 2 * max_depth exceeds the 40 generated dimensions");
        uint32_t m = 0;
        const uint32_t vh = (p->view_height != 0 && p->view_height < ctx->height) ? p->view_height : ctx->height;
        while ((1u << m) < std::max(ctx->width, vh)) ++m;
        if (m > TRC_SOBOL_MAX_LOG2RES) return trc_fail(ctx, TRC_ERR_UNSUPPORTED, "TRC_FLAG_SOBOL: frame too large");
        if (sobol_m) *sobol_m = m;
    }
    if (env_light) return trc_env_light_build(ctx);
    if (mesh_lights) return trc_mesh_light_build(ctx);
    return TRC_OK;
}

constexpr uint32_t kCoalesceBelow = 8, kCoalesceUpTo = 16;
trc_status trc_flush(trc_ctx* ctx) {
    if (!ctx) return TRC_OK;
    TRC_TRY(trc_refit_settle(ctx));
    if (!ctx->has_deferred) return TRC_OK;
    ctx->has_deferred = false;
    const trc_params q = ctx->deferred;
    const uint64_t calls = ctx->deferred_calls;
    const trc_status st = render_pass(ctx, &q, false);
    if (st == TRC_OK && calls > 1) ctx->launches += calls - 1;
    if (st != TRC_OK) {
        ctx->error = "kept launch of " + std::to_string(calls) + " trc_render call(s), frames " + std::to_string(q.frame0) + " .. " +
                     std::to_string(q.frame0 + q.spp - 1) + " (" + std::to_string(q.spp) + " samples per pixel), did not run: " + ctx->error;
    }
    return st;
}
extern "C" {
trc_status trc_render(trc_ctx* ctx, const trc_params* p) {
    TRC_TRY(render_check(ctx, p));
    const bool candidate = p->spp > 0 && p->spp < kCoalesceBelow && !(p->flags & TRC_FLAG_COLLECT_STATS) && !ctx->knobs.no_coalesce;
    if (ctx->has_deferred) {
        trc_params& d = ctx->deferred;
        const bool continues = candidate && p->frame0 == d.frame0 + d.spp && p->max_depth == d.max_depth && p->integrator == d.integrator &&
                               p->tile_rank == d.tile_rank && p->tile_nranks == d.tile_nranks && p->flags == d.flags && p->view_height == d.view_height;
        if (continues) {
            d.spp += p->spp;
            ctx->deferred_calls++;
            return d.spp >= kCoalesceUpTo ? trc_flush(ctx) : TRC_OK;
        }
        TRC_TRY(trc_flush(ctx));
    }
    if (candidate) { ctx->deferred = *p; ctx->deferred_calls = 1; ctx->has_deferred = true; return TRC_OK; }
    return render_pass(ctx, p, false);
}

}

static void launch_params(const trc_ctx* ctx, const trc_params* p, KRender& kp) {
    kp.ks = ctx->ks;
    if (ctx->knobs.descend_min > 0) kp.ks.sc.descend_min = (uint32_t)ctx->knobs.descend_min;
    kp.cam = ctx->cam;
    kp.ambient[0] = ctx->ambient[0]; kp.ambient[1] = ctx->ambient[1]; kp.ambient[2] = ctx->ambient[2];
    kp.env_rgb = ctx->d_envmap; kp.env_w = ctx->env_w; kp.env_h = ctx->env_h;
    if (ctx->tex_active()) { kp.tex_texels = ctx->d_tex_texels; kp.tex_desc = ctx->d_tex_desc; kp.n_tex = ctx->n_tex; }
    kp.fr.rng = ctx->d_rng; kp.fr.accum = ctx->d_accum; kp.fr.width = ctx->width; kp.fr.height = ctx->height;
    kp.spp = p->spp; kp.max_depth = p->max_depth; kp.frame0 = p->frame0;
    kp.view_height = (p->view_height != 0 && p->view_height < ctx->height) ? p->view_height : ctx->height;
    kp.stats = ctx->d_stats;
    kp.block_cost = (p->flags & TRC_FLAG_COLLECT_STATS) ? ctx->d_cost_scratch : ctx->d_block_cost;
    kp.cost_div = std::max(1u, 4u * std::min(p->spp, 1u << 28));
    kp.density = ctx->d_density;
    kp.dinfo = ctx->dinfo;
    kp.occupancy = ctx->d_occupancy;
}

static trc_status launch_geometry(trc_ctx* ctx, const trc_params* p, RenderLaunch& r) {
    const uint32_t nranks = p->tile_nranks ? p->tile_nranks : 1;
    uint32_t blk_shift = 3;
    r.blocks8 = (uint64_t)((ctx->width + 7) / 8) * ((ctx->height + 7) / 8) / nranks;
    r.fits = ctx->width <= 65535u * 4u && ctx->height <= 65535u * 4u;
    if ((p->flags & TRC_FLAG_SMALL_BLOCKS) && r.fits) blk_shift = 2;
    if (ctx->knobs.force_blk_shift > 0) blk_shift = std::min(3u, (uint32_t)ctx->knobs.force_blk_shift - 1u);
    TRC_TRY(trc_ensure_tiles(ctx, nranks, p->tile_rank, p->view_height, blk_shift));
    KRender& kp = r.kp;
    kp.tiles = ctx->d_tiles;
    kp.blk_shift = blk_shift;
    kp.n_tiles = ctx->n_tiles;
    kp.strip = 1;
    if (!r.stats) {
        uint32_t want = p->spp <= 2 ? 3u : p->spp < 8 ? 2u : 1u;
        if (ctx->knobs.strip_len > 0) want = (uint32_t)ctx->knobs.strip_len;
        const uint32_t slots = (uint32_t)ctx->cu_count * 16u;
        const uint32_t room = ctx->n_tiles / (slots + slots / 2u);
        kp.strip = std::max(1u, std::min(want, room));
        if (ctx->knobs.strip_force > 0) kp.strip = std::min((uint32_t)ctx->knobs.strip_force, std::max(1u, ctx->n_tiles));
    }
    r.quarters_ok = kp.strip == 1 && blk_shift == 3;
    kp.cost_stride = r.quarters_ok ? kCostSlots : 1u;
    return TRC_OK;
}

static uint32_t cold_head_spp(const trc_ctx* ctx, const trc_params* p, const RenderLaunch& r, bool inner) {
    const uint32_t head = std::max(kColdHeadSpp, (uint32_t)ctx->knobs.probe_spp);
    const bool cold = !inner && !ctx->cost_valid && !r.stats && !ctx->knobs.no_cold_probe && !(p->flags & TRC_FLAG_FIXED_ORDER) && r.kp.strip == 1 &&
                      p->spp >= 2u * head;
    return cold ? head : 0u;
}
static trc_status render_cold_head(trc_ctx* ctx, const trc_params* p, uint32_t head) {
    trc_params r = *p;
    uint32_t stage = head, done = 0;
    const uint32_t max_stages = ctx->knobs.head_stages > 0 ? (uint32_t)ctx->knobs.head_stages : 3u;
    for (uint32_t k = 0; k < max_stages && p->spp - done >= (k == 0 ? 2u : 4u) * stage; ++k, stage *= 2u) {
        trc_params h = *p;
        h.spp = stage; h.frame0 = p->frame0 + done;
        TRC_TRY(render_pass(ctx, &h, true));
        ctx->launches--;
        if (k == 0) ctx->cost_head_age = 1;
        done += stage;
    }
    r.spp = p->spp - done; r.frame0 = p->frame0 + done;
    return render_pass(ctx, &r, true);
}

static trc_status choose_kernel(trc_ctx* ctx, const trc_params* p, RenderLaunch& r) {
    KRender& kp = r.kp;
    const int integrator = (int)p->integrator;
    const RenderKernels& family = render_family(ctx->lds_scene, p->integrator, ctx->tri_materials);
    const RenderKernel& render_dense = ctx->tri_materials ? trimat::render_dense : ::render_dense;
    r.dense = ctx->lds_scene && integrator == TRC_INTEGRATOR_PATH && !r.stats && !r.sobol && !ctx->tex_active() && kp.strip == 1 && !ctx->knobs.no_dense &&
              ctx->n_tiles >= (uint32_t)TRC_DENSE_MIN_BLOCKS_PER_SLOT * (uint32_t)ctx->cu_count * 4u * render_dense.waves &&
              ((dyn_lds_bytes(kp.ks.sc, false) + (size_t)dense_lds_rows() * kBlock * 4u + 511u) & ~(size_t)511u) * 4u * render_dense.waves <= 160u * 1024u;
    r.wave_slots = (uint32_t)ctx->cu_count * 4u * (uint32_t)(r.dense ? render_dense : family.one[kVariantPlain]).waves;
    uint32_t park_rows = r.dense ? dense_lds_rows() : 0u;
    const bool mem_plan = !r.stats && !ctx->lds_scene;
    if (mem_plan && !ctx->knobs.no_pwg && kp.strip == 1 && ctx->lds_prefix_ok) {
        r.pwg_waves = (uint32_t)pwg_waves(integrator);
        park_rows = pwg_park_rows(integrator);
        r.pwg = plan_pwg_lds(ctx, kp.ks.sc, r.pwg_waves, (uint32_t)pwg_per_cu(integrator), hybrid_stack(integrator), pwg_stack_lds_levels(integrator), park_rows);
        if (!r.pwg) park_rows = 0u;
    }
    const bool tex = ctx->tex_active();
    const RenderVariant variant = r.light == Light::Mesh ? (tex ? kVariantMeshTex : kVariantMesh) : r.light == Light::Env ? (tex ? kVariantEnvTex : kVariantEnv)
                                : tex ? kVariantTex : r.sobol ? kVariantSobol : r.stats ? kVariantStats : kVariantPlain;
    r.kern = r.dense ? render_dense : (r.pwg ? family.pwg : kp.strip > 1 ? family.strip : family.one)[variant];
    if (!r.kern.fn) return trc_fail(ctx, TRC_ERR_UNSUPPORTED, "no render kernel for this integrator, flags and launch shape");
    ctx->last_kernel.shape = r.dense ? 3u : r.pwg ? 2u : kp.strip > 1 ? 1u : 0u;
    ctx->last_kernel.variant = r.dense ? (uint32_t)kVariantPlain : (uint32_t)variant;
    ctx->last_kernel.lds_resident = ctx->lds_scene ? 1u : 0u;
    ctx->last_kernel.tri_materials = ctx->tri_materials ? 1u : 0u;
    ctx->last_kernel.strip = kp.strip;
    ctx->last_kernel.count++;
    if (mem_plan && !r.pwg) plan_launch_lds(ctx, kp.ks.sc, (uint32_t)r.kern.waves, hybrid_stack(integrator));
    r.lds = r.pwg ? ((size_t)kp.ks.sc.lds_dwords + (size_t)r.pwg_waves * (kp.ks.sc.stack_lds + park_rows) * kBlock) * 4
                  : dyn_lds_bytes(kp.ks.sc, r.stats) + (r.dense ? (size_t)park_rows * kBlock * 4 : 0u);
    return TRC_OK;
}

static trc_status launch_buffers(trc_ctx* ctx, const trc_params* p, RenderLaunch& r) {
    KRender& kp = r.kp;
    if (r.sobol) {
        TRC_TRY(ensure_sobol_tables(ctx, kp.sobol_m));
        kp.sobol32 = ctx->d_sobol32;
        kp.sobol_vdc = ctx->d_sobol_vdc;
    }
    if (r.pwg) {
        r.block = 64u * r.pwg_waves;
        r.grid = std::min((uint32_t)ctx->cu_count * (uint32_t)pwg_per_cu((int)p->integrator), (r.grid_cap + r.pwg_waves - 1) / r.pwg_waves);
    } else r.grid = kp.strip > 1 ? (ctx->n_tiles + kp.strip - 1) / kp.strip : r.grid_cap;
    if (!r.stats && !ctx->lds_scene) {
        const size_t rows = kp.ks.sc.stack_ovf_rows;
        const size_t need = rows * kBlock * sizeof(uint32_t) * (r.pwg ? (size_t)r.grid * r.pwg_waves : (size_t)r.grid_cap);
        TRC_TRY(trc_grow_buffer(ctx, ctx->d_stack_ovf, ctx->stack_ovf_bytes, need, "hipMalloc traversal-stack overflow rows"));
        kp.stack_ovf = ctx->d_stack_ovf;
    }
    const size_t memo_rows = r.stats || r.sobol || r.light != Light::None ? 0u : r.pwg ? pwg_memo_rows((int)p->integrator) : (r.dense && TRC_REPLAY_DENSE_GLOBAL) ? (size_t)TRC_REPLAY_DENSE : 0u;
    if (memo_rows) {
        const size_t need = memo_rows * kBlock * sizeof(uint32_t) * (r.pwg ? (size_t)r.grid * r.pwg_waves : (size_t)r.grid_cap);
        TRC_TRY(trc_grow_buffer(ctx, ctx->d_memo, ctx->memo_bytes, need, "hipMalloc primary-replay memo rows"));
        kp.memo = ctx->d_memo;
    }
    kp.replay = ctx->knobs.no_primary_replay ? 0u : (uint32_t)(ctx->knobs.replay_min_lanes > 0 ? ctx->knobs.replay_min_lanes : TRC_REPLAY_MIN_LANES);
    kp.replay_chain = (uint32_t)(ctx->knobs.replay_chain > 0 ? ctx->knobs.replay_chain : TRC_REPLAY_CHAIN);
    if (r.pwg) {
        if (!ctx->d_queue && hipMalloc((void**)&ctx->d_queue, sizeof(uint32_t)) != hipSuccess) return trc_fail(ctx, TRC_ERR_OOM, "hipMalloc block queue");
        HIP_TRY(ctx, hipMemsetAsync(ctx->d_queue, 0, sizeof(uint32_t), ctx->stream));
        kp.queue = ctx->d_queue;
    }
    return TRC_OK;
}

static trc_status timed_launch(trc_ctx* ctx, const RenderLaunch& r) {
    HIP_TRY(ctx, hipGetLastError());
    hipEvent_t e0 = trc_get_event(ctx), e1 = trc_get_event(ctx);
    auto give_back = [&]() { if (e0) ctx->event_pool.push_back(e0); if (e1) ctx->event_pool.push_back(e1); };
    if (!e0 || !e1) { give_back(); return trc_fail(ctx, TRC_ERR_HIP, "hipEventCreate failed"); }
    hipError_t le = hipEventRecord(e0, ctx->stream);
    if (le == hipSuccess) le = launch_render(ctx, r);
    if (le == hipSuccess) le = hipEventRecord(e1, ctx->stream);
    if (le != hipSuccess) { give_back(); return trc_fail(ctx, TRC_ERR_HIP, std::string("k_render launch: ") + hipGetErrorString(le)); }
    ctx->pending.emplace_back(e0, e1);
    ctx->launches++;
    return TRC_OK;
}

static trc_status render_pass(trc_ctx* ctx, const trc_params* p, bool inner) {
    RenderLaunch r;
    TRC_TRY(render_check(ctx, p, &r.kp.sobol_m));
    if (p->spp == 0) return TRC_OK;
    TRC_TRY(trc_refit_settle(ctx));
    HIP_TRY(ctx, hipSetDevice(ctx->device));
    trc_collect_finished_events(ctx);
    r.stats = (p->flags & TRC_FLAG_COLLECT_STATS) != 0;
    r.sobol = (p->flags & TRC_FLAG_SOBOL) != 0;
    r.light = (p->flags & TRC_FLAG_MESH_LIGHTS) ? Light::Mesh : (p->flags & TRC_FLAG_ENV_LIGHT) ? Light::Env : Light::None;
    if (r.light == Light::Env) r.el = trc_env_light_view(ctx);
    if (r.light == Light::Mesh) r.ml = trc_mesh_light_view(ctx);
    TRC_TRY(launch_geometry(ctx, p, r));
    if (ctx->n_tiles == 0) return TRC_OK;
    if (trc_dyn_lds_bytes(ctx, r.stats) > 160 * 1024) return trc_fail(ctx, TRC_ERR_UNSUPPORTED, "traversal stack exceeds the 160 KB LDS of a CU");
    launch_params(ctx, p, r.kp);
    drop_stale_costs(ctx, p, r);
    if (const uint32_t head = cold_head_spp(ctx, p, r, inner)) return render_cold_head(ctx, p, head);
    TRC_TRY(choose_kernel(ctx, p, r));
    TRC_TRY(schedule_blocks(ctx, p, r));
    TRC_TRY(launch_buffers(ctx, p, r));
    return timed_launch(ctx, r);
}

extern "C" {
trc_status trc_debug_primary_replays(trc_ctx* ctx, uint64_t* out) {
    TRC_TRY(trc_flush(ctx));
    if (!ctx || !out) return TRC_ERR_INVALID_ARG;
    HIP_TRY(ctx, hipSetDevice(ctx->device));
    unsigned long long h[kStatCount];
    TRC_TRY(trc_read_stats_sum(ctx, h, kStatCount));
    *out = h[kStatReplays];
    return TRC_OK;
}

trc_status trc_debug_launch_shape(trc_ctx* ctx, trc_launch_shape* out) {
    TRC_TRY(trc_flush(ctx));
    if (!ctx || !out) return TRC_ERR_INVALID_ARG;
    std::memset(out, 0, sizeof *out);
    HIP_TRY(ctx, hipSetDevice(ctx->device));
    int khz = 0;
    if (hipDeviceGetAttribute(&khz, hipDeviceAttributeClockRate, ctx->device) != hipSuccess || khz <= 0) khz = 2400000;
    out->clock_mhz = khz / 1000.0;
    out->wave_slots = ctx->last_wave_slots;
    const uint32_t n = ctx->cost_strip > 1 ? (ctx->n_tiles + ctx->cost_strip - 1) / ctx->cost_strip : ctx->n_tiles;
    if (n == 0 || !ctx->d_block_cost || !ctx->last_cost_div) return TRC_OK;
    HIP_TRY(ctx, hipStreamSynchronize(ctx->stream));
    const uint32_t stride = ctx->cost_quarters ? kCostSlots : 1u;
    std::vector<uint32_t> c((size_t)n * stride), sp(n, 0u), qs((size_t)n * 4u, 0u);
    TRC_TRY(trc_copy_to_host(ctx, c.data(), ctx->d_block_cost, c.size() * 4, ctx->stream));
    if (stride != 1u && ctx->split_live) {
        TRC_TRY(trc_copy_to_host(ctx, sp.data(), ctx->d_split, (size_t)n * 4, ctx->stream));
        TRC_TRY(trc_copy_to_host(ctx, qs.data(), ctx->d_qsplit, (size_t)n * 16, ctx->stream));
    }
    uint64_t sum = 0, longest = 0;
    uint32_t entries = 0;
    auto item = [&](uint32_t v) { sum += v; longest = std::max<uint64_t>(longest, v); entries++; };
    for (uint32_t i = 0; i < n; ++i) {
        const uint32_t* q = &c[(size_t)i * stride];
        if (!sp[i]) { item(q[0]); continue; }
        for_each_part(qs.data(), i, [&](uint32_t slot) { item(q[slot]); });
    }
    const double to_ms = (double)ctx->last_cost_div / ((double)khz);
    out->entries = entries;
    out->longest_entry_ms = (double)longest * to_ms;
    out->sum_entries_ms = (double)sum * to_ms;
    out->work_over_slots_ms = out->wave_slots ? out->sum_entries_ms / out->wave_slots : 0.0;
    return TRC_OK;
}

}
```

### tracer_amd/device.py

```python
import ctypes as C
import os

import numpy as np

from . import abi

_LIB = None
_LIB_FAST = None
_LIB_HOOKS = None


class TracerError(RuntimeError):
    def __init__(self, what, status, detail=""):
        super().__init__(f"{what}: trc_status {status}" + (f" ({detail})" if detail else ""))
        self.status = status


def lib_path():
    return os.environ.get("TRC_AMD_LIB") or os.path.join(os.path.dirname(os.path.abspath(__file__)), "lib", "libtracer_amd.so")


def fast_lib_path():
    return os.path.join(os.path.dirname(os.path.abspath(__file__)), "lib", "libtracer_amd_fast.so")


def hooks_lib_path():
    return os.path.join(os.path.dirname(os.path.abspath(__file__)), "lib", "libtracer_amd_hooks.so")


def lib(fast_math=False, hooks=False):
    global _LIB, _LIB_FAST, _LIB_HOOKS
    if hooks:
        if _LIB_HOOKS is None:
            _LIB_HOOKS = _load(hooks_lib_path(), hooks=True)
            assert _LIB_HOOKS.trc_has_test_hooks() == 1
        return _LIB_HOOKS
    if fast_math:
        if _LIB_FAST is None:
            _LIB_FAST = _load(fast_lib_path())
            assert _LIB_FAST.trc_build_flavor() == b"fast-math"
        return _LIB_FAST
    if _LIB is None:
        _LIB = _load(lib_path())
    return _LIB


def _load(path, hooks=False):
    if not os.path.exists(path):
        raise RuntimeError(f"{path} is missing: the HIP extension is not built "
                           f"(run `make hip` or __graft_entry__.build()); there is no CPU fallback")
    L = C.CDLL(path)
    vp, u32, u64, i32 = C.c_void_p, C.c_uint32, C.c_uint64, C.c_int32
    L.trc_abi_version.restype = u32
    L.trc_build_flavor.restype = C.c_char_p
    L.trc_status_string.argtypes = [i32]
    L.trc_status_string.restype = C.c_char_p
    L.trc_last_error.argtypes = [vp]
    L.trc_last_error.restype = C.c_char_p
    L.trc_create.argtypes = [C.c_int, C.POINTER(vp)]
    L.trc_destroy.argtypes = [vp]
    L.trc_destroy.restype = None
    L.trc_upload_scene.argtypes = [vp, C.POINTER(abi.Scene)]
    L.trc_set_environment_map.argtypes = [vp, u32, u32, vp]
    L.trc_tonemap.argtypes = [vp, vp, C.POINTER(C.c_float)]
    L.trc_upload_density.argtypes = [vp, C.POINTER(abi.GridDensityInfo), vp]
    L.trc_upload_scene_lbvh.argtypes = [vp, C.POINTER(abi.Scene)]
    L.trc_upload_scene_sah.argtypes = [vp, C.POINTER(abi.Scene)]
    L.trc_upload_scene_device.argtypes = [vp, C.POINTER(abi.Scene), u32]
    L.trc_download_bvh.argtypes = [vp, C.POINTER(abi.BVH), u32, C.POINTER(u32)]
    L.trc_lbvh_info.argtypes = [vp, C.POINTER(u32), C.POINTER(u32), C.POINTER(C.c_float)]
    L.trc_set_camera.argtypes = [vp, C.POINTER(abi.Camera)]
    L.trc_set_environment.argtypes = [vp, C.POINTER(C.c_float)]
    L.trc_resize.argtypes = [vp, u32, u32]
    L.trc_seed.argtypes = [vp, u64]
    for name in ("trc_upload_rng", "trc_download_rng", "trc_upload_accum", "trc_download_accum"):
        getattr(L, name).argtypes = [vp, vp]
    L.trc_clear_accum.argtypes = [vp]
    L.trc_render.argtypes = [vp, C.POINTER(abi.Params)]
    L.trc_synchronize.argtypes = [vp]
    L.trc_trace_rays.argtypes = [vp, vp, C.c_size_t, vp, C.c_int]
    L.trc_get_stats.argtypes = [vp, C.POINTER(abi.Stats)]
    L.trc_reset_stats.argtypes = [vp]
    L.trc_sppm_init.argtypes = [vp, u64]
    L.trc_sppm_frames.argtypes = [vp, u32]
    L.trc_sppm_download.argtypes = [vp, vp, vp, vp, vp, C.POINTER(abi.Complex)]
    L.trc_device_info.argtypes = [vp, C.c_char_p, C.c_size_t, C.POINTER(C.c_int), C.POINTER(C.c_size_t)]
    L.trc_group_unique_id.argtypes = [C.POINTER(C.c_uint8)]
    L.trc_group_init.argtypes = [vp, C.POINTER(C.c_uint8), C.c_int, C.c_int]
    L.trc_group_reduce_accum.argtypes = [vp, C.c_int]
    L.trc_group_reduce_accum_async.argtypes = [vp, C.c_int]
    L.trc_group_allreduce_mean_accum.argtypes = [vp]
    L.trc_group_compose_samples.argtypes = [vp, C.c_int, u32]
    L.trc_group_compose_samples_async.argtypes = [vp, C.c_int, u32]
    L.trc_shard_seed.argtypes = [u64, u32]
    L.trc_device_pci_bus_id.argtypes = [vp, C.c_char_p, C.c_size_t]
    L.trc_download_composed.argtypes = [vp, vp]
    L.trc_group_finalize.argtypes = [vp]
    L.trc_group_set_collectives.argtypes = [vp, vp, C.c_int, C.c_int]
    L.trc_debug_set.argtypes = [vp, C.c_char_p, C.c_int]
    L.trc_debug_block_costs.argtypes = [vp, vp, vp, u32, C.POINTER(u32), C.POINTER(u32)]
    L.trc_debug_launch_shape.argtypes = [vp, C.POINTER(abi.LaunchShape)]
    L.trc_debug_primary_replays.argtypes = [vp, C.POINTER(u64)]
    L.trc_denoise_default_params.argtypes = [C.POINTER(abi.DenoiseParams)]
    L.trc_denoise.argtypes = [vp, C.POINTER(abi.DenoiseParams)]
    L.trc_download_denoised.argtypes = [vp, vp]
    L.trc_tonemap_denoised.argtypes = [vp, vp, C.POINTER(C.c_float)]
    L.trc_download_gbuffer.argtypes = [vp, vp]
    L.trc_denoise_reset.argtypes = [vp]
    L.trc_upload_textures.argtypes = [vp, C.POINTER(abi.Image), u32]
    L.trc_upload_triangle_materials.argtypes = [vp, vp, u32]
    L.trc_update_vertices.argtypes = [vp, vp, u32, u32]
    L.trc_debug_refit_ms.argtypes = [vp, C.POINTER(C.c_float)]
    L.trc_pose_vertices.argtypes = [vp, C.POINTER(abi.Pose), u32]
    L.trc_download_vertices.argtypes = [vp, vp, u32, u32]
    L.trc_debug_pose_overflows.argtypes = [vp, C.POINTER(u32)]
    if hooks:
        L.trc_debug_profile.argtypes = [vp, C.POINTER(C.c_uint64), u32]
        L.trc_sppm_hash_cells.argtypes = [vp, vp, C.c_size_t, C.c_float, vp]
        L.trc_div_by_test.argtypes = [vp, vp, vp, C.c_size_t, vp, vp]
        L.trc_unary_test.argtypes = [vp, u32, u32, C.c_uint64, C.POINTER(C.c_uint64), C.POINTER(u32)]
        L.trc_debug_denoise_state.argtypes = [vp, vp, vp, vp]
        L.trc_texture_sample_test.argtypes = [vp, u32, vp, C.c_size_t, vp]
        L.trc_debug_env_tables.argtypes = [vp, vp, vp, vp, C.POINTER(C.c_double), C.POINTER(C.c_float)]
        L.trc_env_light_test.argtypes = [vp, vp, C.c_size_t, vp, vp, C.c_size_t, vp]
        L.trc_debug_mesh_light_tables.argtypes = [vp, vp, vp, vp, C.POINTER(C.c_double), C.POINTER(u32)]
        L.trc_mesh_light_test.argtypes = [vp, vp, vp, C.c_size_t, vp, vp]
        L.trc_debug_last_kernel.argtypes = [vp, C.POINTER(abi.KernelChoice)]
        for name in abi.HOOK_SYMBOLS:
            getattr(L, name).restype = i32
    L.trc_has_test_hooks.restype = C.c_int
    for name in abi.DEVICE_SYMBOLS:
        f = getattr(L, name)
        if name not in ("trc_abi_version", "trc_build_flavor", "trc_has_test_hooks", "trc_status_string", "trc_last_error", "trc_destroy", "trc_shard_seed",
                        "trc_denoise_default_params"):
            f.restype = i32
    L.trc_shard_seed.restype = u64
    L.trc_denoise_default_params.restype = None
    if L.trc_abi_version() != abi.TRC_ABI_VERSION:
        raise RuntimeError("libtracer_amd.so ABI version mismatch")
    return L


def make_poses(poses):
    arr = (abi.Pose * len(poses))()
    for k, (first, count, model, normal) in enumerate(poses):
        arr[k].first, arr[k].count = int(first), int(count)
        for name, m in (("model_matrix", model), ("normal_matrix", normal)):
            m = np.asarray(m, dtype=np.float32).reshape(4, 4)
            cols = getattr(arr[k], name).columns
            for c in range(4):
                cols[c].x, cols[c].y, cols[c].z, cols[c].w = (float(m[r, c]) for r in range(4))
    return arr


def group_unique_id():
    buf = (C.c_uint8 * abi.TRC_UNIQUE_ID_BYTES)()
    st = lib().trc_group_unique_id(buf)
    if st != abi.OK:
        raise TracerError("trc_group_unique_id", st)
    return bytes(buf)


class Tracer:

    def __init__(self, device=0, fast_math=False, hooks=False):
        self._L = lib(fast_math, hooks)
        self._env_shape = (0, 0)
        self._h = C.c_void_p()
        st = self._L.trc_create(device, C.byref(self._h))
        if st != abi.OK:
            self._h = None
            raise TracerError(f"trc_create(device={device})", st, self._L.trc_status_string(st).decode())
        self.width = self.height = 0
        self._n_vertex = 0

    def _check(self, st, what):
        if st != abi.OK:
            raise TracerError(what, st, self._L.trc_last_error(self._h).decode())

    def close(self):
        if getattr(self, "_h", None):
            self._L.trc_destroy(self._h)
            self._h = None

    __del__ = close

    def __enter__(self):
        return self

    def __exit__(self, *exc):
        self.close()

    def upload_scene(self, scene_view):
        self._check(self._L.trc_upload_scene(self._h, C.byref(scene_view)), "trc_upload_scene")
        self._n_vertex = scene_view.n_vertex

    def set_environment_map(self, rgb):
        if rgb is None:
            self._check(self._L.trc_set_environment_map(self._h, 0, 0, None), "trc_set_environment_map")
            self._env_shape = (0, 0)
            return
        assert rgb.dtype == np.float32 and rgb.ndim == 3 and rgb.shape[2] == 3 and rgb.flags.c_contiguous
        self._check(self._L.trc_set_environment_map(self._h, rgb.shape[1], rgb.shape[0], rgb.ctypes.data),
                    "trc_set_environment_map")
        self._env_shape = rgb.shape[:2]

    def upload_textures(self, images):
        images = [np.ascontiguousarray(a, dtype=np.float32) for a in (images or [])]
        for a in images:
            assert a.ndim == 3 and a.shape[2] == 3, a.shape
        arr = (abi.Image * max(1, len(images)))()
        for k, a in enumerate(images):
            arr[k].width, arr[k].height = a.shape[1], a.shape[0]
            arr[k].rgb = a.ctypes.data_as(C.POINTER(C.c_float))
        self._check(self._L.trc_upload_textures(self._h, arr if images else None, len(images)), "trc_upload_textures")

    def upload_triangle_materials(self, material):
        if material is None:
            self._check(self._L.trc_upload_triangle_materials(self._h, None, 0), "trc_upload_triangle_materials")
            return
        m = np.ascontiguousarray(material, dtype=np.uint32).ravel()
        buf = m if m.size else np.zeros(1, np.uint32)
        self._check(self._L.trc_upload_triangle_materials(self._h, buf.ctypes.data, m.size), "trc_upload_triangle_materials")

    def update_vertices(self, vertices, first=0):
        v = np.ascontiguousarray(vertices, dtype=np.float32).reshape(-1, 8)
        buf = v if v.size else np.zeros((1, 8), np.float32)
        self._check(self._L.trc_update_vertices(self._h, buf.ctypes.data, first, v.shape[0]), "trc_update_vertices")

    def pose_vertices(self, poses):
        if not (isinstance(poses, C.Array) and poses._type_ is abi.Pose):
            poses = make_poses(poses)
        self._check(self._L.trc_pose_vertices(self._h, poses if len(poses) else None, len(poses)), "trc_pose_vertices")

    def download_vertices(self, first=0, count=None):
        if count is None:
            count = max(self._n_vertex - first, 0)
        out = np.empty((max(count, 0), 8), dtype=np.float32)
        buf = out if out.size else np.zeros((1, 8), np.float32)
        self._check(self._L.trc_download_vertices(self._h, buf.ctypes.data, first, count), "trc_download_vertices")
        return out

    def pose_overflows(self):
        n = C.c_uint32(0)
        self._check(self._L.trc_debug_pose_overflows(self._h, C.byref(n)), "trc_debug_pose_overflows")
        return n.value

    def refit_ms(self):
        ms = C.c_float(0)
        self._check(self._L.trc_debug_refit_ms(self._h, C.byref(ms)), "trc_debug_refit_ms")
        return ms.value

    def texture_sample(self, index, uv):
        uv = np.ascontiguousarray(uv, dtype=np.float32).reshape(-1, 2)
        out = np.empty((uv.shape[0], 3), dtype=np.float32)
        self._check(self._L.trc_texture_sample_test(self._h, index, uv.ctypes.data, uv.shape[0], out.ctypes.data), "trc_texture_sample_test")
        return out

    def env_tables(self):
        H, W = self._env_shape
        weight = np.empty((H, W), np.float32)
        rows = np.empty((H, W, 2), np.uint32)
        marg = np.empty((H, 2), np.uint32)
        total, ms = C.c_double(), C.c_float()
        self._check(self._L.trc_debug_env_tables(self._h, weight.ctypes.data, rows.ctypes.data, marg.ctypes.data, C.byref(total), C.byref(ms)),
                    "trc_debug_env_tables")
        return dict(weight=weight, rows=rows, marg=marg, total=total.value, build_ms=ms.value)

    def env_light_test(self, draws=None, dirs=None):
        d = np.ascontiguousarray(np.zeros((0, 6), np.uint32) if draws is None else draws, dtype=np.uint32).reshape(-1, 6)
        v = np.ascontiguousarray(np.zeros((0, 3), np.float32) if dirs is None else dirs, dtype=np.float32).reshape(-1, 3)
        out = np.empty((d.shape[0], 4), np.float32)
        pdf = np.empty(v.shape[0], np.float32)
        self._check(self._L.trc_env_light_test(self._h, d.ctypes.data, d.shape[0], out.ctypes.data, v.ctypes.data, v.shape[0], pdf.ctypes.data),
                    "trc_env_light_test")
        return out, pdf

    def mesh_light_tables(self, n_triangles):
        total, n = C.c_double(), C.c_uint32()
        self._check(self._L.trc_debug_mesh_light_tables(self._h, None, None, None, C.byref(total), C.byref(n)), "trc_debug_mesh_light_tables")
        alias = np.zeros((n.value, 2), np.uint32)
        tri = np.zeros(n.value, np.uint32)
        pdfA = np.zeros(n_triangles, np.float32)
        self._check(self._L.trc_debug_mesh_light_tables(self._h, alias.ctypes.data if n.value else None, tri.ctypes.data if n.value else None,
                                                        pdfA.ctypes.data if n_triangles else None, C.byref(total), C.byref(n)),
                    "trc_debug_mesh_light_tables")
        return dict(alias=alias, tri=tri, pdfA=pdfA, total=total.value, n_lights=n.value)

    def mesh_light_test(self, draws, pos):
        d = np.ascontiguousarray(draws, dtype=np.uint32).reshape(-1, 4)
        v = np.ascontiguousarray(pos, dtype=np.float32).reshape(-1, 3)
        assert d.shape[0] == v.shape[0]
        tri = np.empty(d.shape[0], np.uint32)
        out = np.empty((d.shape[0], 7), np.float32)
        self._check(self._L.trc_mesh_light_test(self._h, d.ctypes.data, v.ctypes.data, d.shape[0], tri.ctypes.data, out.ctypes.data),
                    "trc_mesh_light_test")
        return tri, out

    def tonemap(self):
        out = np.empty((self.height, self.width, 4), dtype=np.uint8)
        e = C.c_float(0)
        self._check(self._L.trc_tonemap(self._h, out.ctypes.data, C.byref(e)), "trc_tonemap")
        return out, e.value

    def upload_density(self, info, density):
        if density is None:
            self._check(self._L.trc_upload_density(self._h, None, None), "trc_upload_density")
            return
        assert density.dtype == np.float32 and density.flags.c_contiguous
        self._check(self._L.trc_upload_density(self._h, C.byref(info), density.ctypes.data), "trc_upload_density")

    def upload_scene_lbvh(self, leaves_view):
        self._check(self._L.trc_upload_scene_lbvh(self._h, C.byref(leaves_view)), "trc_upload_scene_lbvh")
        self._n_vertex = leaves_view.n_vertex

    def upload_scene_sah(self, leaves_view):
        self._check(self._L.trc_upload_scene_sah(self._h, C.byref(leaves_view)), "trc_upload_scene_sah")
        self._n_vertex = leaves_view.n_vertex

    def upload_scene_device(self, view, flags):
        self._check(self._L.trc_upload_scene_device(self._h, C.byref(view), flags), "trc_upload_scene_device")
        self._n_vertex = view.n_vertex

    def download_bvh(self):
        n = C.c_uint32(0)
        self._check(self._L.trc_download_bvh(self._h, None, 0, C.byref(n)), "trc_download_bvh")
        out = (abi.BVH * n.value)()
        self._check(self._L.trc_download_bvh(self._h, out, n.value, C.byref(n)), "trc_download_bvh")
        return out

    def lbvh_info(self):
        n, h, ms = C.c_uint32(0), C.c_uint32(0), C.c_float(0)
        self._check(self._L.trc_lbvh_info(self._h, C.byref(n), C.byref(h), C.byref(ms)), "trc_lbvh_info")
        return n.value, h.value, ms.value

    def set_camera(self, camera):
        self._check(self._L.trc_set_camera(self._h, C.byref(camera)), "trc_set_camera")

    def set_environment(self, rgb):
        self._check(self._L.trc_set_environment(self._h, (C.c_float * 3)(*rgb)), "trc_set_environment")

    def resize(self, width, height):
        self._check(self._L.trc_resize(self._h, width, height), "trc_resize")
        self.width, self.height = width, height

    def seed(self, seed):
        self._check(self._L.trc_seed(self._h, seed), "trc_seed")

    def upload_rng(self, rng):
        assert rng.dtype == np.uint32 and rng.shape == (self.height, self.width, 4) and rng.flags.c_contiguous
        self._check(self._L.trc_upload_rng(self._h, rng.ctypes.data), "trc_upload_rng")

    def download_rng(self):
        out = np.empty((self.height, self.width, 4), dtype=np.uint32)
        self._check(self._L.trc_download_rng(self._h, out.ctypes.data), "trc_download_rng")
        return out

    def upload_accum(self, accum):
        assert accum.dtype == np.float32 and accum.shape == (self.height, self.width, 4) and accum.flags.c_contiguous
        self._check(self._L.trc_upload_accum(self._h, accum.ctypes.data), "trc_upload_accum")

    def download_accum(self):
        out = np.empty((self.height, self.width, 4), dtype=np.float32)
        self._check(self._L.trc_download_accum(self._h, out.ctypes.data), "trc_download_accum")
        return out

    def clear_accum(self):
        self._check(self._L.trc_clear_accum(self._h), "trc_clear_accum")

    def render(self, spp=1, max_depth=8, integrator=abi.INTEGRATOR_PATH, frame0=0, tile_rank=0, tile_nranks=1,
               collect_stats=False, view_height=0, fixed_order=False, sobol=False, small_blocks=None, env_light=False,
               mesh_lights=False):
        flags = ((abi.FLAG_COLLECT_STATS if collect_stats else 0) | (abi.FLAG_FIXED_ORDER if fixed_order else 0) |
                 (abi.FLAG_SOBOL if sobol else 0) | (abi.FLAG_ENV_LIGHT if env_light else 0) | (abi.FLAG_MESH_LIGHTS if mesh_lights else 0) |
                 (0 if small_blocks is None else (abi.FLAG_SMALL_BLOCKS if small_blocks else abi.FLAG_LARGE_BLOCKS)))
        prm = abi.Params(spp=spp, max_depth=max_depth, integrator=integrator, frame0=frame0, tile_rank=tile_rank,
                         tile_nranks=tile_nranks, flags=flags, view_height=view_height)
        self._check(self._L.trc_render(self._h, C.byref(prm)), "trc_render")

    def synchronize(self):
        self._check(self._L.trc_synchronize(self._h), "trc_synchronize")

    def trace_rays(self, rays, any_hit=False, production=False):
        from .dtypes import HIT_DTYPE, RAY_DTYPE
        assert rays.dtype == RAY_DTYPE and rays.flags.c_contiguous
        hits = np.zeros(len(rays), dtype=HIT_DTYPE)
        self._check(self._L.trc_trace_rays(self._h, rays.ctypes.data, len(rays), hits.ctypes.data,
                                           (abi.TRACE_ANY_HIT if any_hit else 0) | (abi.TRACE_PRODUCTION if production else 0)),
                    "trc_trace_rays")
        return hits

    def denoise_params(self, **overrides):
        p = abi.DenoiseParams()
        self._L.trc_denoise_default_params(C.byref(p))
        if overrides.pop("demodulate", False):
            p.flags |= abi.DENOISE_DEMODULATE
        for k, v in overrides.items():
            setattr(p, k, v)
        return p

    def denoise(self, params=None, **overrides):
        p = params if params is not None else self.denoise_params(**overrides)
        self._check(self._L.trc_denoise(self._h, C.byref(p)), "trc_denoise")

    def download_denoised(self):
        out = np.empty((self.height, self.width, 4), dtype=np.float32)
        self._check(self._L.trc_download_denoised(self._h, out.ctypes.data), "trc_download_denoised")
        return out

    def tonemap_denoised(self):
        out = np.empty((self.height, self.width, 4), dtype=np.uint8)
        e = C.c_float(0)
        self._check(self._L.trc_tonemap_denoised(self._h, out.ctypes.data, C.byref(e)), "trc_tonemap_denoised")
        return out, e.value

    def download_gbuffer(self):
        from .dtypes import GBUFFER_DTYPE
        out = np.empty((self.height, self.width), dtype=GBUFFER_DTYPE)
        self._check(self._L.trc_download_gbuffer(self._h, out.ctypes.data), "trc_download_gbuffer")
        return out

    def denoise_reset(self):
        self._check(self._L.trc_denoise_reset(self._h), "trc_denoise_reset")

    def denoise_state(self):
        planes = [np.empty((self.height, self.width, 4), dtype=np.float32) for _ in range(3)]
        self._check(self._L.trc_debug_denoise_state(self._h, *(p.ctypes.data for p in planes)), "trc_debug_denoise_state")
        return tuple(planes)

    def stats(self):
        s = abi.Stats()
        self._check(self._L.trc_get_stats(self._h, C.byref(s)), "trc_get_stats")
        return s

    PROFILE_SITES = ["loop", "box_step", "square", "sphere", "cube", "triangle", "shade", "lambert", "metal",
                     "beckmann_sample", "beckmann_eval", "path_end"]

    def debug_profile(self):
        n = len(self.PROFILE_SITES)
        buf = (C.c_uint64 * (3 * n))()
        self._check(self._L.trc_debug_profile(self._h, buf, n), "trc_debug_profile")
        return {s: (buf[3 * i], buf[3 * i + 1], buf[3 * i] / (64.0 * buf[3 * i + 1]) if buf[3 * i + 1] else 0.0,
                    buf[3 * i + 2]) for i, s in enumerate(self.PROFILE_SITES)}

    def reset_stats(self):
        self._check(self._L.trc_reset_stats(self._h), "trc_reset_stats")

    def device_info(self):
        name = C.create_string_buffer(256)
        cu, mem = C.c_int(), C.c_size_t()
        self._check(self._L.trc_device_info(self._h, name, 256, C.byref(cu), C.byref(mem)), "trc_device_info")
        return {"name": name.value.decode(), "cu_count": cu.value, "hbm_bytes": mem.value}

    def sppm_init(self, photon_seed):
        self._check(self._L.trc_sppm_init(self._h, photon_seed), "trc_sppm_init")

    def sppm_frames(self, n_frames=1):
        self._check(self._L.trc_sppm_frames(self._h, n_frames), "trc_sppm_frames")

    def sppm_hash_cells(self, cells, hash_scale):
        cells = np.ascontiguousarray(cells, dtype=np.float32).reshape(-1, 3)
        out = np.empty(len(cells), dtype=np.float32)
        self._check(self._L.trc_sppm_hash_cells(self._h, cells.ctypes.data, len(cells), float(hash_scale), out.ctypes.data),
                    "trc_sppm_hash_cells")
        return out

    def sppm_download(self):
        from .dtypes import CAMREC_DTYPE, PHOTON_DTYPE
        n = abi.PHOTON_HASHN
        cam = np.zeros(self.width * self.height, dtype=CAMREC_DTYPE)
        pho = np.zeros(n * n, dtype=PHOTON_DTYPE)
        mark = np.zeros((n, n, 4), dtype=np.float32)
        count = np.zeros((n, n), dtype=np.float32)
        cx = abi.Complex()
        self._check(self._L.trc_sppm_download(self._h, cam.ctypes.data, pho.ctypes.data, mark.ctypes.data,
                                              count.ctypes.data, C.byref(cx)), "trc_sppm_download")
        return cam, pho, mark, count, cx

    def group_init(self, unique_id, nranks, rank):
        buf = (C.c_uint8 * abi.TRC_UNIQUE_ID_BYTES).from_buffer_copy(unique_id)
        self._check(self._L.trc_group_init(self._h, buf, nranks, rank), "trc_group_init")

    def group_reduce_accum(self, root=0):
        self._check(self._L.trc_group_reduce_accum(self._h, root), "trc_group_reduce_accum")

    def group_allreduce_mean_accum(self):
        self._check(self._L.trc_group_allreduce_mean_accum(self._h), "trc_group_allreduce_mean_accum")

    def group_compose_samples(self, root=0, sample_groups=None):
        self._check(self._L.trc_group_compose_samples(self._h, root, sample_groups or 0), "trc_group_compose_samples")

    def group_compose_samples_async(self, root=0, sample_groups=None):
        self._check(self._L.trc_group_compose_samples_async(self._h, root, sample_groups or 0), "trc_group_compose_samples_async")

    def pci_bus_id(self):
        buf = C.create_string_buffer(64)
        self._check(self._L.trc_device_pci_bus_id(self._h, buf, 64), "trc_device_pci_bus_id")
        return buf.value.decode()

    def group_reduce_accum_async(self, root=0):
        self._check(self._L.trc_group_reduce_accum_async(self._h, root), "trc_group_reduce_accum_async")

    def download_composed(self):
        out = np.empty((self.height, self.width, 4), dtype=np.float32)
        self._check(self._L.trc_download_composed(self._h, out.ctypes.data), "trc_download_composed")
        return out

    def set_collectives(self, table, nranks, rank):
        self._coll = table
        self._check(self._L.trc_group_set_collectives(self._h, C.byref(table.table) if table is not None else None, nranks, rank),
                    "trc_group_set_collectives")

    def debug_set(self, knob, value):
        self._check(self._L.trc_debug_set(self._h, knob.encode(), int(value)), "trc_debug_set")

    def last_kernel(self):
        k = abi.KernelChoice()
        self._check(self._L.trc_debug_last_kernel(self._h, C.byref(k)), "trc_debug_last_kernel")
        return dict(shape=abi.KERNEL_SHAPES[k.shape], variant=abi.KERNEL_VARIANTS[k.variant], lds_resident=bool(k.lds_resident),
                    triangle_materials=bool(k.triangle_materials), strip=int(k.strip), launches=int(k.launches))

    def div_by_test(self, a, b):
        a = np.ascontiguousarray(a, dtype=np.float32); b = np.ascontiguousarray(b, dtype=np.float32)
        assert a.shape == b.shape and a.ndim == 1
        fast, plain = np.empty((len(a), 3), np.float32), np.empty((len(a), 3), np.float32)
        self._check(self._L.trc_div_by_test(self._h, a.ctypes.data, b.ctypes.data, len(a), fast.ctypes.data, plain.ctypes.data), "trc_div_by_test")
        return fast, plain

    def block_costs(self):
        n, bs = C.c_uint32(0), C.c_uint32(0)
        self._check(self._L.trc_debug_block_costs(self._h, None, None, 0, C.byref(n), C.byref(bs)), "trc_debug_block_costs")
        tiles, costs = np.zeros(n.value, np.uint32), np.zeros(n.value, np.uint32)
        self._check(self._L.trc_debug_block_costs(self._h, tiles.ctypes.data, costs.ctypes.data, n.value, C.byref(n), C.byref(bs)),
                    "trc_debug_block_costs")
        return tiles, costs, bs.value

    def unary_test(self, op, first_bits=0, count=1 << 32):
        n, first = C.c_uint64(0), C.c_uint32(0)
        self._check(self._L.trc_unary_test(self._h, op, first_bits, count, C.byref(n), C.byref(first)), "trc_unary_test")
        return n.value, first.value

    def launch_shape(self):
        s = abi.LaunchShape()
        self._check(self._L.trc_debug_launch_shape(self._h, C.byref(s)), "trc_debug_launch_shape")
        return {k: getattr(s, k) for k, _ in abi.LaunchShape._fields_}

    def primary_replays(self):
        n = C.c_uint64(0)
        self._check(self._L.trc_debug_primary_replays(self._h, C.byref(n)), "trc_debug_primary_replays")
        return n.value

    def group_finalize(self):
        self._check(self._L.trc_group_finalize(self._h), "trc_group_finalize")
```

Baseline: 14100.

## Pack dense memo into one word and size LDS by queried occupancy

Dense replay memo rows shrink from eight to seven by packing hit/ends/none state, material, tag type and index into one 32-bit word. The LDS plan now asks the runtime for resident workgroups, then shrinks the scene-prefix share and stack levels until the register-limited occupancy is reached. Dense eligibility also uses queried occupancy instead of a fixed granule formula. A debug hook reports residency. The aim is more resident waves and more LDS for BVH nodes, at the cost of extra occupancy queries, pack/unpack work, and a fallback path when material or index values exceed the packed limits.

After: 14820, median of 6. +5.1%, better.

```diff
diff --git a/include/tracer_test_hooks.h b/include/tracer_test_hooks.h
--- a/include/tracer_test_hooks.h
+++ b/include/tracer_test_hooks.h
@@ -31,6 +31,14 @@
 } trc_kernel_choice;
 trc_status trc_debug_last_kernel(trc_ctx* ctx, trc_kernel_choice* out);
 
+
+typedef struct trc_residency {
+    uint32_t cu_count, block, waves, planned_per_cu, planned_with, per_cu;
+    uint64_t lds_bytes;
+    uint32_t lds_static_bytes, per_cu_block1280, dense_memo_rows, reserved;
+} trc_residency;
+trc_status trc_debug_last_residency(trc_ctx* ctx, trc_residency* out);
+
 #ifdef __cplusplus
 }
 #endif
diff --git a/tracer_amd/abi.py b/tracer_amd/abi.py
--- a/tracer_amd/abi.py
+++ b/tracer_amd/abi.py
@@ -207,6 +207,12 @@
                 ("strip", C.c_uint32), ("launches", C.c_uint32)]
 
 
+class Residency(C.Structure):
+    _fields_ = [("cu_count", C.c_uint32), ("block", C.c_uint32), ("waves", C.c_uint32), ("planned_per_cu", C.c_uint32),
+                ("planned_with", C.c_uint32), ("per_cu", C.c_uint32), ("lds_bytes", C.c_uint64),
+                ("lds_static_bytes", C.c_uint32), ("per_cu_block1280", C.c_uint32), ("dense_memo_rows", C.c_uint32), ("reserved", C.c_uint32)]
+
+
 KERNEL_SHAPES = ("one", "strip", "pwg", "dense")
 KERNEL_VARIANTS = ("plain", "stats", "sobol", "tex", "env", "env_tex", "mesh", "mesh_tex")
 
@@ -247,7 +253,8 @@
     "trc_pose_vertices", "trc_download_vertices", "trc_debug_pose_overflows",
 ]
 HOOK_SYMBOLS = ["trc_debug_profile", "trc_sppm_hash_cells", "trc_div_by_test", "trc_unary_test", "trc_debug_denoise_state", "trc_texture_sample_test",
-                "trc_debug_env_tables", "trc_env_light_test", "trc_debug_mesh_light_tables", "trc_mesh_light_test", "trc_debug_last_kernel"]
+                "trc_debug_env_tables", "trc_env_light_test", "trc_debug_mesh_light_tables", "trc_mesh_light_test", "trc_debug_last_kernel",
+                "trc_debug_last_residency"]
 HOST_SYMBOLS = [
     "trc_host_build_node", "trc_host_build_tree", "trc_host_tree_depth", "trc_host_make_camera",
     "trc_host_prepare_camera", "trc_host_fill_rng", "trc_host_scene_create", "trc_host_scene_create_leaves", "trc_host_scene_destroy",
diff --git a/tracer_amd/csrc/trc_ctx.hpp b/tracer_amd/csrc/trc_ctx.hpp
--- a/tracer_amd/csrc/trc_ctx.hpp
+++ b/tracer_amd/csrc/trc_ctx.hpp
@@ -197,6 +197,7 @@
     bool cost_valid = false; uint32_t cost_strip = 1;
     uint32_t last_cost_div = 0, last_wave_slots = 0;
     struct LastKernel { uint32_t shape = 0, variant = 0, lds_resident = 0, tri_materials = 0, strip = 0, count = 0; } last_kernel;
+    struct LastFit { const void* fn = nullptr; uint32_t block = 0, waves = 0, planned_per_cu = 0, per_cu = 0; size_t lds = 0; } last_fit;
     trc_params deferred{}; bool has_deferred = false; uint64_t deferred_calls = 0;
     int cost_head_age = 0;
     bool cost_fresh_next = false;
@@ -263,6 +264,8 @@
         int strip_force = 0;
     } knobs;
     std::vector<const void*> lds_granted;
+    struct Residency { const void* fn; uint32_t block; size_t lds; uint32_t per_cu; };
+    std::vector<Residency> residency;
 
     bool grouped() const { return comm != nullptr || coll_active; }
 };
diff --git a/tracer_amd/csrc/trc_hooks.hip b/tracer_amd/csrc/trc_hooks.hip
--- a/tracer_amd/csrc/trc_hooks.hip
+++ b/tracer_amd/csrc/trc_hooks.hip
@@ -3,6 +3,7 @@
 #include <string>
 
 #include "trc_ctx.hpp"
+#include "trc_render_config.hpp"
 
 extern "C" int trc_has_test_hooks(void) {
 #ifdef TRC_TEST_HOOKS
@@ -91,6 +92,24 @@
     out->strip = k.strip; out->launches = k.count;
     return TRC_OK;
 }
+trc_status trc_debug_last_residency(trc_ctx* ctx, trc_residency* out) {
+    TRC_TRY(trc_flush(ctx));
+    if (!ctx || !out) return TRC_ERR_INVALID_ARG;
+    const trc_ctx::LastFit& f = ctx->last_fit;
+    *out = trc_residency{};
+    if (!f.fn) return TRC_OK;
+    HIP_TRY(ctx, hipSetDevice(ctx->device));
+    int now = 0;
+    HIP_TRY(ctx, hipOccupancyMaxActiveBlocksPerMultiprocessor(&now, f.fn, (int)f.block, f.lds));
+    hipFuncAttributes attr{};
+    HIP_TRY(ctx, hipFuncGetAttributes(&attr, f.fn));
+    out->cu_count = (uint32_t)ctx->cu_count; out->block = f.block; out->waves = f.waves; out->planned_per_cu = f.planned_per_cu;
+    out->planned_with = f.per_cu; out->per_cu = now > 0 ? (uint32_t)now : 0u; out->lds_bytes = (uint64_t)f.lds;
+    out->lds_static_bytes = (uint32_t)attr.sharedSizeBytes;
+    out->per_cu_block1280 = trc_lds_workgroups((uint32_t)(f.lds + attr.sharedSizeBytes), 1280u, 160u * 1024u);
+    out->dense_memo_rows = ctx->last_kernel.shape == 3u ? (uint32_t)TRC_REPLAY_DENSE : 0u;
+    return TRC_OK;
+}
 
 trc_status trc_div_by_test(trc_ctx* ctx, const float* a, const float* b, size_t n, float* fast, float* plain) {
     if (!ctx || (n && (!a || !b || !fast || !plain))) return TRC_ERR_INVALID_ARG;
diff --git a/tracer_amd/csrc/trc_lds_fit.hpp b/tracer_amd/csrc/trc_lds_fit.hpp
--- /dev/null
+++ b/tracer_amd/csrc/trc_lds_fit.hpp
@@ -0,0 +1,39 @@
+#pragma once
+
+#include <stdint.h>
+
+#if defined(__HIPCC__)
+#define TRC_FIT_FN __host__ __device__ __forceinline__
+#else
+#define TRC_FIT_FN inline
+#endif
+
+TRC_FIT_FN uint32_t trc_lds_workgroups(uint32_t bytes, uint32_t granule, uint32_t lds_per_cu) {
+    if (granule == 0u) return 0u;
+    const uint32_t granted = (bytes + granule - 1u) / granule * granule;
+    return granted ? lds_per_cu / granted : 0xFFFFFFFFu;
+}
+
+constexpr uint32_t kPackIndexBits = 20u, kPackMatBits = 8u, kPackTypeBits = 2u;
+constexpr uint32_t kPackHit = 0x80000000u, kPackSameSide = 0x40000000u, kPackEnds = 0x40000000u;
+constexpr uint32_t kPackCountMax = 0x3FFFFFFFu;
+constexpr uint32_t kPackMatMax = (1u << kPackMatBits) - 1u, kPackIndexMax = (1u << kPackIndexBits) - 1u;
+static_assert(2u + kPackTypeBits + kPackMatBits + kPackIndexBits == 32u, "packed memo word: kind 2 + type 2 + material 8 + index 20 bits");
+static_assert(kPackCountMax >= 65535u, "the replay count of a lost record");
+
+TRC_FIT_FN bool trc_memo_packable(uint32_t material, uint32_t tag_type, uint32_t tag_index) {
+    return material <= kPackMatMax && tag_type < (1u << kPackTypeBits) && tag_index <= kPackIndexMax;
+}
+TRC_FIT_FN uint32_t trc_memo_pack_hit(uint32_t material, bool same_side, uint32_t tag_type, uint32_t tag_index) {
+    return kPackHit | (same_side ? kPackSameSide : 0u) | (tag_type << (kPackMatBits + kPackIndexBits)) | (material << kPackIndexBits) | tag_index;
+}
+TRC_FIT_FN uint32_t trc_memo_pack_none(uint32_t replays) { return replays < kPackCountMax ? replays : kPackCountMax; }
+TRC_FIT_FN uint32_t trc_memo_pack_ends() { return kPackEnds; }
+TRC_FIT_FN bool trc_memo_is_none(uint32_t w) { return (w >> 30) == 0u; }
+TRC_FIT_FN bool trc_memo_is_ends(uint32_t w) { return (w >> 30) == 1u; }
+TRC_FIT_FN bool trc_memo_is_hit(uint32_t w) { return (w & kPackHit) != 0u; }
+TRC_FIT_FN uint32_t trc_memo_count(uint32_t w) { return w & kPackCountMax; }
+TRC_FIT_FN bool trc_memo_same_side(uint32_t w) { return (w & kPackSameSide) != 0u; }
+TRC_FIT_FN uint32_t trc_memo_material(uint32_t w) { return (w >> kPackIndexBits) & kPackMatMax; }
+TRC_FIT_FN uint32_t trc_memo_tag_type(uint32_t w) { return (w >> (kPackMatBits + kPackIndexBits)) & ((1u << kPackTypeBits) - 1u); }
+TRC_FIT_FN uint32_t trc_memo_tag_index(uint32_t w) { return w & kPackIndexMax; }
diff --git a/tracer_amd/csrc/trc_render_config.hpp b/tracer_amd/csrc/trc_render_config.hpp
--- a/tracer_amd/csrc/trc_render_config.hpp
+++ b/tracer_amd/csrc/trc_render_config.hpp
@@ -1,6 +1,7 @@
 #pragma once
 
 #include "trc_ctx.hpp"
+#include "trc_lds_fit.hpp"
 
 #ifndef TRC_MIS_HYBRID
 #define TRC_MIS_HYBRID 1
@@ -78,10 +79,11 @@
 static_assert((TRC_PARK_PATH == 0 || TRC_PARK_PATH == 8 || TRC_PARK_PATH == 10) && (TRC_PARK_MIS == 0 || TRC_PARK_MIS == 8 || TRC_PARK_MIS == 10) &&
               (TRC_PARK_VOLUME == 0 || TRC_PARK_VOLUME == 8 || TRC_PARK_VOLUME == 10) && (TRC_PARK_DENSE == 0 || TRC_PARK_DENSE == 8 || TRC_PARK_DENSE == 10), "park rows: 0, 8 or 10");
 enum : uint32_t { kMemoPx = 0, kMemoPy, kMemoPz, kMemoNx, kMemoNy, kMemoNz, kMemoTag, kMemoMat, kMemoU, kMemoV };
+constexpr uint32_t kMemoWord = kMemoTag;
 constexpr uint32_t kMemoNone = 0xFFFFFFFFu;
 constexpr uint32_t kMemoSameSide = 0x80000000u;
 #ifndef TRC_REPLAY_DENSE
-#define TRC_REPLAY_DENSE 8
+#define TRC_REPLAY_DENSE 7
 #endif
 #ifndef TRC_REPLAY_DENSE_GLOBAL
 #define TRC_REPLAY_DENSE_GLOBAL 0
@@ -95,7 +97,7 @@
 #ifndef TRC_REPLAY_CHAIN
 #define TRC_REPLAY_CHAIN 1
 #endif
-static_assert((TRC_REPLAY_DENSE == 0 || TRC_REPLAY_DENSE == 8 || TRC_REPLAY_DENSE == 10) && (TRC_REPLAY_PWG_PATH == 0 || TRC_REPLAY_PWG_PATH == 10), "memo rows: 0, 8 or 10 (10 wherever image textures may be live)");
+static_assert((TRC_REPLAY_DENSE == 0 || TRC_REPLAY_DENSE == 7 || TRC_REPLAY_DENSE == 8 || TRC_REPLAY_DENSE == 10) && (TRC_REPLAY_PWG_PATH == 0 || TRC_REPLAY_PWG_PATH == 10), "memo rows: 0, 7 (dense), 8 or 10 (10 wherever image textures may be live)");
 constexpr uint32_t dense_lds_rows() { return (uint32_t)TRC_PARK_DENSE + (TRC_REPLAY_DENSE_GLOBAL ? 0u : (uint32_t)TRC_REPLAY_DENSE); }
 constexpr uint32_t pwg_memo_rows(int integrator) { return integrator == TRC_INTEGRATOR_PATH ? (uint32_t)TRC_REPLAY_PWG_PATH : 0u; }
 #ifndef TRC_PWG_STACK_LDS_PATH
diff --git a/tracer_amd/csrc/trc_render_kernels.hpp b/tracer_amd/csrc/trc_render_kernels.hpp
--- a/tracer_amd/csrc/trc_render_kernels.hpp
+++ b/tracer_amd/csrc/trc_render_kernels.hpp
@@ -50,6 +50,7 @@
                                              const LightTables<LIGHT>* tables = nullptr, uint32_t* memo = nullptr) {
     static_assert(MEMO == 0 || (INTEGRATOR == TRC_INTEGRATOR_PATH && !STATS && !SOBOL && LIGHT == Light::None), "primary replay: tracePath production kernels");
     static_assert(MEMO == 0 || MEMO == 10 || !TEX, "an image texture reads rec.uv: 10 memo rows");
+    constexpr bool kPacked = MEMO == 7;
     uint32_t replays = 0;
     const uint64_t t_start = clock64();
     const uint32_t entry = kp.order ? kp.order[slot] : slot;
@@ -113,23 +114,25 @@
             path_begin(ps, cast_ray(kp.cam, u, v, rng), kp.max_depth);
             if constexpr (MEMO != 0) {
                 if (replay_on && s != 0u) {
-                    const uint32_t mat = memo[kMemoMat * kBlock];
-                    if (mat != kMemoNone) {
+                    const uint32_t mat = memo[(kPacked ? kMemoWord : kMemoMat) * kBlock];
+                    if (kPacked ? !trc_memo_is_none(mat) : mat != kMemoNone) {
                         if (at_eye(ps.ray.o)) {
-                            const uint32_t tag = memo[kMemoTag * kBlock];
+                            const uint32_t tag = kPacked ? (trc_memo_is_ends(mat) ? kTagNone : (trc_memo_tag_type(mat) << kTagIndexBits) | trc_memo_tag_index(mat))
+                                                         : memo[kMemoTag * kBlock];
                             if (tag == kTagNone) terminal = true;
                             else {
                                 ps.rec.p = f3(memo_f(kMemoPx), memo_f(kMemoPy), memo_f(kMemoPz));
                                 ps.rec.gn = f3(memo_f(kMemoNx), memo_f(kMemoNy), memo_f(kMemoNz));
-                                ps.rec.sn = (mat & kMemoSameSide) ? ps.rec.gn : -ps.rec.gn;
-                                ps.rec.material = mat & ~kMemoSameSide;
+                                ps.rec.sn = (kPacked ? trc_memo_same_side(mat) : (mat & kMemoSameSide) != 0u) ? ps.rec.gn : -ps.rec.gn;
+                                ps.rec.material = kPacked ? trc_memo_material(mat) : mat & ~kMemoSameSide;
                                 ps.rec.tag = tag;
                                 if constexpr (MEMO >= 10) { ps.rec.uv.x = memo_f(kMemoU); ps.rec.uv.y = memo_f(kMemoV); }
                                 have = true;
                             }
                             bump(n_rays);
                         } else {
-                            memo[kMemoMat * kBlock] = kMemoNone; memo[kMemoTag * kBlock] = s - 1u;
+                            if constexpr (kPacked) memo[kMemoWord * kBlock] = trc_memo_pack_none(s - 1u);
+                            else { memo[kMemoMat * kBlock] = kMemoNone; memo[kMemoTag * kBlock] = s - 1u; }
                         }
                     }
                 }
@@ -187,7 +190,9 @@
                 if (ends) { mat = 0u; tag = kTagNone; }
                 else {
                     const bool uv_read = MEMO < 10 && (ps.rec.tag >> kTagIndexBits) >= 2u && mat_tex(cx.sh, ps.rec.material) == kTexChecker;
-                    if (!uv_read && ps.rec.material < kMemoSameSide - 1u) {
+                    const bool fits = kPacked ? trc_memo_packable(ps.rec.material, ps.rec.tag >> kTagIndexBits, ps.rec.tag & kTagIndexMask)
+                                              : ps.rec.material < kMemoSameSide - 1u;
+                    if (!uv_read && fits) {
                         const bool same = __float_as_uint(ps.rec.sn.x) == __float_as_uint(ps.rec.gn.x);
                         mat = ps.rec.material | (same ? kMemoSameSide : 0u); tag = ps.rec.tag;
                         memo[kMemoPx * kBlock] = __float_as_uint(ps.rec.p.x); memo[kMemoPy * kBlock] = __float_as_uint(ps.rec.p.y);
@@ -198,7 +203,10 @@
                     }
                 }
             }
-            memo[kMemoMat * kBlock] = mat; memo[kMemoTag * kBlock] = tag;
+            if constexpr (kPacked) {
+                memo[kMemoWord * kBlock] = mat == kMemoNone ? trc_memo_pack_none(0u) : tag == kTagNone ? trc_memo_pack_ends()
+                                         : trc_memo_pack_hit(mat & ~kMemoSameSide, (mat & kMemoSameSide) != 0u, tag >> kTagIndexBits, tag & kTagIndexMask);
+            } else { memo[kMemoMat * kBlock] = mat; memo[kMemoTag * kBlock] = tag; }
             return ends;
         };
         uint32_t drained = 0;
@@ -233,7 +241,8 @@
             }
         }
         if constexpr (MEMO != 0) {
-            if (replay_on) replays = memo[kMemoMat * kBlock] != kMemoNone ? kp.spp - 1u : memo[kMemoTag * kBlock];
+            if constexpr (kPacked) { if (replay_on) { const uint32_t w = memo[kMemoWord * kBlock]; replays = trc_memo_is_none(w) ? trc_memo_count(w) : kp.spp - 1u; } }
+            else if (replay_on) replays = memo[kMemoMat * kBlock] != kMemoNone ? kp.spp - 1u : memo[kMemoTag * kBlock];
         }
         if constexpr (PARK) {
             n_paths += kp.spp;
diff --git a/tracer_amd/csrc/trc_render_pass.hip b/tracer_amd/csrc/trc_render_pass.hip
--- a/tracer_amd/csrc/trc_render_pass.hip
+++ b/tracer_amd/csrc/trc_render_pass.hip
@@ -18,22 +18,66 @@
     sc.stack_lds = std::min(sc.stack_depth, std::max(1u, levels));
     sc.stack_ovf_rows = sc.stack_depth - sc.stack_lds;
 }
-static void plan_launch_lds(const trc_ctx* ctx, DScene& sc, uint32_t waves_per_simd, bool hybrid) {
+static hipError_t grant_lds(trc_ctx* ctx, const void* fn, size_t lds) {
+    if (lds <= 64 * 1024 || std::find(ctx->lds_granted.begin(), ctx->lds_granted.end(), fn) != ctx->lds_granted.end()) return hipSuccess;
+    const hipError_t e = hipFuncSetAttribute(fn, hipFuncAttributeMaxDynamicSharedMemorySize, (int)(160 * 1024));
+    if (e == hipSuccess) ctx->lds_granted.push_back(fn);
+    return e;
+}
+
+static trc_status resident_workgroups(trc_ctx* ctx, const void* fn, uint32_t block, size_t lds, uint32_t* per_cu) {
+    for (const trc_ctx::Residency& e : ctx->residency)
+        if (e.fn == fn && e.block == block && e.lds == lds) { *per_cu = e.per_cu; return TRC_OK; }
+    HIP_TRY(ctx, grant_lds(ctx, fn, lds));
+    if (ctx->residency.size() >= 64u) ctx->residency.clear();
+    int n = 0;
+    HIP_TRY(ctx, hipOccupancyMaxActiveBlocksPerMultiprocessor(&n, fn, (int)block, lds));
+    *per_cu = (uint32_t)std::max(n, 0);
+    ctx->residency.push_back({fn, block, lds, *per_cu});
+    return TRC_OK;
+}
+static trc_status resident_by_registers(trc_ctx* ctx, const void* fn, uint32_t block, uint32_t* per_cu) { return resident_workgroups(ctx, fn, block, 0, per_cu); }
+
+constexpr uint32_t kLdsStepDwords = 128;
+
+static trc_status plan_launch_lds(trc_ctx* ctx, DScene& sc, const RenderKernel& kern, bool hybrid) {
     const uint32_t levels = ctx->knobs.stack_lds_levels > 0 ? (uint32_t)ctx->knobs.stack_lds_levels : kStackLdsLevels;
     if (hybrid) set_hybrid_stack(sc, ctx->knobs.no_lds_fit ? std::max(levels, sc.stack_depth) : levels);
-    if (ctx->knobs.no_lds_fit) return;
-    if (!ctx->lds_prefix_ok) return;
-    const uint32_t per_wg = ((160u * 1024u / 4u) / (4u * waves_per_simd)) & ~127u;
-    const uint32_t stack = sc.stack_lds * kBlock;
-    uint32_t room = std::max(per_wg > stack ? per_wg - stack : 0u, sc.off_nodes + kNodeDwords);
-    room = std::min(room, kLdsSceneBytes / 4);
-    sc.n_lds_nodes = std::min(sc.n_nodes, (room - sc.off_nodes) / kNodeDwords);
-    sc.lds_dwords = sc.off_nodes + sc.n_lds_nodes * kNodeDwords;
-}
-
-static bool plan_pwg_lds(const trc_ctx* ctx, DScene& sc, uint32_t waves, uint32_t per_cu, bool hybrid, uint32_t default_levels, uint32_t park_rows) {
+    if (ctx->knobs.no_lds_fit) return TRC_OK;
+    if (!ctx->lds_prefix_ok) return TRC_OK;
+    const uint32_t planned = 4u * (uint32_t)kern.waves;
+    uint32_t want = 0;
+    TRC_TRY(resident_by_registers(ctx, kern.fn, kBlock, &want));
+    want = std::min(want, planned);
+    const uint32_t share = ((160u * 1024u / 4u) / planned) & ~(kLdsStepDwords - 1u);
+    const uint32_t least = sc.off_nodes + kNodeDwords;
+    auto plan_prefix = [&](uint32_t per_wg) {
+        const uint32_t stack = sc.stack_lds * kBlock;
+        uint32_t room = std::max(per_wg > stack ? per_wg - stack : 0u, least);
+        room = std::min(room, kLdsSceneBytes / 4);
+        sc.n_lds_nodes = std::min(sc.n_nodes, (room - sc.off_nodes) / kNodeDwords);
+        sc.lds_dwords = sc.off_nodes + sc.n_lds_nodes * kNodeDwords;
+        return room > least;
+    };
+    plan_prefix(share);
+    const DScene first = sc;
+    for (uint32_t lv = sc.stack_lds;; --lv) {
+        if (lv != first.stack_lds) set_hybrid_stack(sc, lv);
+        for (uint32_t per_wg = share;; per_wg -= kLdsStepDwords) {
+            const bool more = plan_prefix(per_wg);
+            uint32_t fit = 0;
+            TRC_TRY(resident_workgroups(ctx, kern.fn, kBlock, dyn_lds_bytes(sc, false), &fit));
+            if (fit >= want) return TRC_OK;
+            if (!more || per_wg < kLdsStepDwords) break;
+        }
+        if (!hybrid || lv <= 6u || ctx->knobs.stack_lds_levels > 0) break;
+    }
+    sc = first;
+    return TRC_OK;
+}
+
+static bool plan_pwg_share(const trc_ctx* ctx, DScene& sc, uint32_t waves, uint32_t per_wg, bool hybrid, uint32_t default_levels, uint32_t park_rows) {
     uint32_t levels = ctx->knobs.stack_lds_levels > 0 ? (uint32_t)ctx->knobs.stack_lds_levels : default_levels;
-    const uint32_t per_wg = ((160u * 1024u / 4u) / per_cu) & ~127u;
     for (;; --levels) {
         DScene t = sc;
         if (hybrid) set_hybrid_stack(t, levels);
@@ -47,6 +91,12 @@
         if (!hybrid || levels <= 6u || ctx->knobs.stack_lds_levels > 0) return false;
     }
 }
+static size_t pwg_lds_bytes(const DScene& sc, uint32_t waves, uint32_t park_rows) {
+    return ((size_t)sc.lds_dwords + (size_t)waves * (sc.stack_lds + park_rows) * kBlock) * 4;
+}
+static bool plan_pwg_lds(const trc_ctx* ctx, DScene& sc, uint32_t waves, uint32_t per_cu, bool hybrid, uint32_t default_levels, uint32_t park_rows) {
+    return plan_pwg_share(ctx, sc, waves, ((160u * 1024u / 4u) / per_cu) & ~(kLdsStepDwords - 1u), hybrid, default_levels, park_rows);
+}
 
 namespace {
 
@@ -80,11 +130,7 @@
 
 hipError_t launch_render(trc_ctx* ctx, const RenderLaunch& r) {
     const void* const fn = r.kern.fn;
-    if (r.lds > 64 * 1024 && std::find(ctx->lds_granted.begin(), ctx->lds_granted.end(), fn) == ctx->lds_granted.end()) {
-        const hipError_t e = hipFuncSetAttribute(fn, hipFuncAttributeMaxDynamicSharedMemorySize, (int)(160 * 1024));
-        if (e != hipSuccess) return e;
-        ctx->lds_granted.push_back(fn);
-    }
+    if (const hipError_t e = grant_lds(ctx, fn, r.lds); e != hipSuccess) return e;
     KRenderEnv kpe;
     KRenderMesh kpm;
     void* params = const_cast<KRender*>(&r.kp);
@@ -250,10 +296,16 @@
     const int integrator = (int)p->integrator;
     const RenderKernels& family = render_family(ctx->lds_scene, p->integrator, ctx->tri_materials);
     const RenderKernel& render_dense = ctx->tri_materials ? trimat::render_dense : ::render_dense;
+    const bool tex = ctx->tex_active();
+    const RenderVariant variant = r.light == Light::Mesh ? (tex ? kVariantMeshTex : kVariantMesh) : r.light == Light::Env ? (tex ? kVariantEnvTex : kVariantEnv)
+                                : tex ? kVariantTex : r.sobol ? kVariantSobol : r.stats ? kVariantStats : kVariantPlain;
     r.dense = ctx->lds_scene && integrator == TRC_INTEGRATOR_PATH && !r.stats && !r.sobol && !ctx->tex_active() && kp.strip == 1 && !ctx->knobs.no_dense &&
-              ctx->n_tiles >= (uint32_t)TRC_DENSE_MIN_BLOCKS_PER_SLOT * (uint32_t)ctx->cu_count * 4u * render_dense.waves &&
-              ((dyn_lds_bytes(kp.ks.sc, false) + (size_t)dense_lds_rows() * kBlock * 4u + 511u) & ~(size_t)511u) * 4u * render_dense.waves <= 160u * 1024u;
-    r.wave_slots = (uint32_t)ctx->cu_count * 4u * (uint32_t)(r.dense ? render_dense : family.one[kVariantPlain]).waves;
+              ctx->n_tiles >= (uint32_t)TRC_DENSE_MIN_BLOCKS_PER_SLOT * (uint32_t)ctx->cu_count * 4u * render_dense.waves;
+    uint32_t dense_per_cu = 0;
+    if (r.dense) {
+        TRC_TRY(resident_workgroups(ctx, render_dense.fn, kBlock, dyn_lds_bytes(kp.ks.sc, false) + (size_t)dense_lds_rows() * kBlock * 4u, &dense_per_cu));
+        r.dense = dense_per_cu >= 4u * (uint32_t)render_dense.waves;
+    }
     uint32_t park_rows = r.dense ? dense_lds_rows() : 0u;
     const bool mem_plan = !r.stats && !ctx->lds_scene;
     if (mem_plan && !ctx->knobs.no_pwg && kp.strip == 1 && ctx->lds_prefix_ok) {
@@ -262,9 +314,6 @@
         r.pwg = plan_pwg_lds(ctx, kp.ks.sc, r.pwg_waves, (uint32_t)pwg_per_cu(integrator), hybrid_stack(integrator), pwg_stack_lds_levels(integrator), park_rows);
         if (!r.pwg) park_rows = 0u;
     }
-    const bool tex = ctx->tex_active();
-    const RenderVariant variant = r.light == Light::Mesh ? (tex ? kVariantMeshTex : kVariantMesh) : r.light == Light::Env ? (tex ? kVariantEnvTex : kVariantEnv)
-                                : tex ? kVariantTex : r.sobol ? kVariantSobol : r.stats ? kVariantStats : kVariantPlain;
     r.kern = r.dense ? render_dense : (r.pwg ? family.pwg : kp.strip > 1 ? family.strip : family.one)[variant];
     if (!r.kern.fn) return trc_fail(ctx, TRC_ERR_UNSUPPORTED, "no render kernel for this integrator, flags and launch shape");
     ctx->last_kernel.shape = r.dense ? 3u : r.pwg ? 2u : kp.strip > 1 ? 1u : 0u;
@@ -273,9 +322,15 @@
     ctx->last_kernel.tri_materials = ctx->tri_materials ? 1u : 0u;
     ctx->last_kernel.strip = kp.strip;
     ctx->last_kernel.count++;
-    if (mem_plan && !r.pwg) plan_launch_lds(ctx, kp.ks.sc, (uint32_t)r.kern.waves, hybrid_stack(integrator));
-    r.lds = r.pwg ? ((size_t)kp.ks.sc.lds_dwords + (size_t)r.pwg_waves * (kp.ks.sc.stack_lds + park_rows) * kBlock) * 4
+    if (mem_plan && !r.pwg) TRC_TRY(plan_launch_lds(ctx, kp.ks.sc, r.kern, hybrid_stack(integrator)));
+    r.lds = r.pwg ? pwg_lds_bytes(kp.ks.sc, r.pwg_waves, park_rows)
                   : dyn_lds_bytes(kp.ks.sc, r.stats) + (r.dense ? (size_t)park_rows * kBlock * 4 : 0u);
+    const uint32_t per_cu = r.dense ? dense_per_cu : 4u * (uint32_t)family.one[kVariantPlain].waves;
+    r.wave_slots = (uint32_t)ctx->cu_count * per_cu;
+    trc_ctx::LastFit& fit = ctx->last_fit;
+    fit.fn = r.kern.fn; fit.block = r.pwg ? 64u * r.pwg_waves : kBlock; fit.waves = (uint32_t)r.kern.waves; fit.lds = r.lds;
+    fit.planned_per_cu = r.pwg ? (uint32_t)pwg_per_cu(integrator) : 4u * fit.waves;
+    TRC_TRY(resident_workgroups(ctx, fit.fn, fit.block, fit.lds, &fit.per_cu));
     return TRC_OK;
 }
 
diff --git a/tracer_amd/device.py b/tracer_amd/device.py
--- a/tracer_amd/device.py
+++ b/tracer_amd/device.py
@@ -126,6 +126,7 @@
         L.trc_debug_mesh_light_tables.argtypes = [vp, vp, vp, vp, C.POINTER(C.c_double), C.POINTER(u32)]
         L.trc_mesh_light_test.argtypes = [vp, vp, vp, C.c_size_t, vp, vp]
         L.trc_debug_last_kernel.argtypes = [vp, C.POINTER(abi.KernelChoice)]
+        L.trc_debug_last_residency.argtypes = [vp, C.POINTER(abi.Residency)]
         for name in abi.HOOK_SYMBOLS:
             getattr(L, name).restype = i32
     L.trc_has_test_hooks.restype = C.c_int
@@ -520,6 +521,11 @@
         return dict(shape=abi.KERNEL_SHAPES[k.shape], variant=abi.KERNEL_VARIANTS[k.variant], lds_resident=bool(k.lds_resident),
                     triangle_materials=bool(k.triangle_materials), strip=int(k.strip), launches=int(k.launches))
 
+    def last_residency(self):
+        r = abi.Residency()
+        self._check(self._L.trc_debug_last_residency(self._h, C.byref(r)), "trc_debug_last_residency")
+        return {name: int(getattr(r, name)) for name, _ in abi.Residency._fields_}
+
     def div_by_test(self, a, b):
         a = np.ascontiguousarray(a, dtype=np.float32); b = np.ascontiguousarray(b, dtype=np.float32)
         assert a.shape == b.shape and a.ndim == 1
```
